# Wp-Zhang/HandyRec

Measured on NVIDIA B200. Metric: DeepFM train samples/s, higher is better.
Workload: dtype f32

## Files before the change

handyrec_b200/csrc/embedding_bwd.cu:

```cuda
#include <cub/block/block_radix_sort.cuh>
#include <cub/block/block_scan.cuh>

#include <stdlib.h>

#include <algorithm>
#include <new>
#include <vector>

#include "plan.cuh"

namespace hrb {

constexpr int UB_THREADS = 256;
constexpr int UB_IPT = 16;
constexpr int UB_CAP = UB_THREADS * UB_IPT;
constexpr int UB_EXPECT_MAX = 3686;
constexpr int UB_MAX_COLS = 256;
constexpr int UB_MAX_BINS = 256;
constexpr int UB_BINS = 64;
constexpr int UB_STACK = 256;
constexpr int UB_WARPS = UB_THREADS / 32;
constexpr int UB_HELPERS = 4;
constexpr int UB_TILE = 4096;
constexpr int SPLIT_ROUNDS = UB_TILE / UB_WARPS / 32;
constexpr uint32_t UB_INVALID = 0xFFFFFFFFu;
constexpr uint32_t UB_NONE = 0xFFFFFFFEu;
constexpr int UB_SLICE_TARGET = 4096;
constexpr int UB_PARTIAL_LD = 32 * 4 + 4;
constexpr int UB_GATHER = 8;
constexpr int UB_APPLY = 2;

static inline size_t ub_align(size_t x, size_t a = 256) { return (x + a - 1) / a * a; }

__global__ void __launch_bounds__(256) bwd_prep_kernel(const FieldDev* __restrict__ fields, const int32_t* __restrict__ pos_field,
                                                      int32_t pos_cols, const int32_t* __restrict__ ids, int64_t ids_ld, int64_t batch,
                                                      int64_t ldT, uint32_t* __restrict__ idsT) {
  __shared__ uint32_t tile[32][33];
  const int tx = threadIdx.x & 31, ty = threadIdx.x >> 5;
  const int64_t b0 = (int64_t)blockIdx.x * 32;
  const int c0 = blockIdx.y * 32;
  const int c = c0 + tx;
  int ids_col = 0, pool = 0;
  int64_t rows = 0;
  if (c < pos_cols) {
    const FieldDev& f = fields[pos_field[c]];
    ids_col = f.ids_col + (c - f.pos_col);
    pool = f.pool;
    rows = f.rows;
  }
  for (int r = ty; r < 32; r += 8) {
    const int64_t b = b0 + r;
    uint32_t v = UB_INVALID;
    if (b < batch && c < pos_cols) {
      const int32_t id = ids[b * ids_ld + ids_col];
      const bool valid = (pool == HRB_POOL_NONE || id != 0) && id >= 0 && (int64_t)id < rows;
      if (valid) v = (uint32_t)id;
    }
    tile[r][tx] = v;
  }
  __syncthreads();
  for (int r = ty; r < 32; r += 8) {
    const int cc = c0 + r;
    const int64_t b = b0 + tx;
    if (cc < pos_cols && b < ldT) idsT[(int64_t)cc * ldT + b] = tile[tx][r];
  }
}

__global__ void __launch_bounds__(256) bwd_scale_kernel(const FieldDev* __restrict__ fields, int32_t n_fields,
                                                       const int32_t* __restrict__ ids, int64_t ids_ld, int64_t batch,
                                                       float* __restrict__ scale) {
  const int64_t total = batch * n_fields;
  for (int64_t i = blockIdx.x * (int64_t)blockDim.x + threadIdx.x; i < total; i += (int64_t)gridDim.x * blockDim.x) {
    const int64_t b = i / n_fields;
    const int fi = (int)(i - b * n_fields);
    const FieldDev& f = fields[fi];
    float s = 1.0f;
    if (f.pool == HRB_POOL_MEAN) {
      const int32_t* idp = ids + b * ids_ld + f.ids_col;
      int cnt = 0;
      for (int l = 0; l < f.seq_len; ++l) {
        const int32_t id = idp[l];
        cnt += (id != 0 && id >= 0 && (int64_t)id < f.rows);
      }
      s = cnt > 0 ? __fdiv_rn(1.0f, (float)cnt) : 0.f;
    }
    scale[i] = s;
  }
}

struct SplitArgs {
  const TableSplitDev* splits;
  const TileDev* tiles;
  const uint32_t* idsT;
  int64_t ldT;
  uint32_t* tile_cnt;
  uint32_t* list_cnt;
  uint32_t* list_off;
  uint32_t* ent_row;
  uint32_t* ent_pos;
};

template <bool SCATTER>
__global__ void __launch_bounds__(UB_THREADS) split_kernel(SplitArgs a) {
  __shared__ uint32_t wcnt[UB_WARPS][UB_MAX_BINS];
  const int tid = threadIdx.x, lane = tid & 31, w = tid >> 5;
  const TileDev tile = a.tiles[blockIdx.x];
  const TableSplitDev ts = a.splits[tile.table];
  for (int i = tid; i < UB_WARPS * UB_MAX_BINS; i += UB_THREADS) (&wcnt[0][0])[i] = 0;
  __syncthreads();
  const uint32_t* colp = a.idsT + (int64_t)tile.pos_col * a.ldT;
  const int64_t b0 = (int64_t)tile.chunk * UB_TILE + w * (UB_TILE / UB_WARPS);
  uint32_t packed[SPLIT_ROUNDS];
  uint32_t idv[SPLIT_ROUNDS];
#pragma unroll
  for (int k = 0; k < SPLIT_ROUNDS; ++k) {
    const int64_t b = b0 + k * 32 + lane;
    idv[k] = b < a.ldT ? __ldg(colp + b) : UB_INVALID;
  }
#pragma unroll
  for (int k = 0; k < SPLIT_ROUNDS; ++k) {
    const uint32_t id = idv[k];
    const uint32_t bin = id == UB_INVALID ? UB_INVALID : id >> ts.shift;
    const uint32_t peers = __match_any_sync(0xffffffffu, bin);
    const int leader = __ffs(peers) - 1;
    uint32_t base = 0;
    if (bin != UB_INVALID && lane == leader) {
      base = wcnt[w][bin];
      wcnt[w][bin] = base + __popc(peers);
    }
    if (SCATTER) {
      base = __shfl_sync(0xffffffffu, base, leader);
      packed[k] = bin == UB_INVALID ? UB_INVALID : (bin << 16) | (base + __popc(peers & ((1u << lane) - 1u)));
    }
    __syncwarp();
  }
  __syncthreads();
  uint32_t* tc = a.tile_cnt + (size_t)blockIdx.x * UB_MAX_BINS;
  if (!SCATTER) {
    for (int u = tid; u < ts.n_bins; u += UB_THREADS) {
      uint32_t t = 0;
#pragma unroll
      for (int ww = 0; ww < UB_WARPS; ++ww) t += wcnt[ww][u];
      tc[u] = t;
    }
    return;
  }
  for (int u = tid; u < ts.n_bins; u += UB_THREADS) {
    uint32_t run = tc[u];
#pragma unroll
    for (int ww = 0; ww < UB_WARPS; ++ww) {
      const uint32_t t = wcnt[ww][u];
      wcnt[ww][u] = run;
      run += t;
    }
  }
  __syncthreads();
  const uint32_t mask = (1u << ts.shift) - 1u;
#pragma unroll
  for (int k = 0; k < SPLIT_ROUNDS; ++k) {
    if (packed[k] == UB_INVALID) continue;
    const int64_t b = b0 + k * 32 + lane;
    const uint32_t id = idv[k];
    const uint32_t dst = wcnt[w][packed[k] >> 16] + (packed[k] & 0xFFFFu);
    a.ent_row[dst] = id & mask;
    a.ent_pos[dst] = ((uint32_t)tile.col_local << 24) | (uint32_t)b;
  }
}

__global__ void __launch_bounds__(UB_MAX_BINS) split_scan_kernel(SplitArgs a) {
  __shared__ uint32_t tot[UB_MAX_BINS];
  const TableSplitDev ts = a.splits[blockIdx.x];
  const int u = threadIdx.x;
  uint32_t run = 0;
  if (u < ts.n_bins) {
    for (int t = 0; t < ts.n_tiles; ++t) {
      uint32_t* p = a.tile_cnt + (size_t)(ts.first_tile + t) * UB_MAX_BINS + u;
      const uint32_t c = *p;
      *p = run;
      run += c;
    }
  }
  tot[u] = u < ts.n_bins ? run : 0;
  __syncthreads();
  for (int off = 1; off < UB_MAX_BINS; off <<= 1) {
    const uint32_t v = u >= off ? tot[u - off] : 0;
    __syncthreads();
    tot[u] += v;
    __syncthreads();
  }
  if (u < ts.n_bins) {
    const uint32_t base = ts.ent_base + tot[u] - run;
    a.list_cnt[ts.first_list + u] = run;
    a.list_off[ts.first_list + u] = base;
    for (int t = 0; t < ts.n_tiles; ++t) a.tile_cnt[(size_t)(ts.first_tile + t) * UB_MAX_BINS + u] += base;
  }
}

struct UnitArgs {
  const UnitDev* units;
  const TableDev* tables;
  const ColDev* cols;
  const int32_t* col_start;
  const uint32_t* list_cnt;
  const uint32_t* list_off;
  const uint32_t* ent_row;
  const uint32_t* ent_pos;
  const float* dout;
  int64_t dout_ld;
  const float* scale;
  int32_t n_fields;
  int32_t n_units;
  hrb_opt_params opt;
  float lr_t;
  float* partials;
  int32_t debug;
};
#ifdef HRB_DEVTOOLS
#define HRB_UDBG(b) (a.debug & (b))
#else
#define HRB_UDBG(b) 0
#endif

template <int G>
struct UnitSmem {
  typedef cub::BlockRadixSort<uint32_t, UB_THREADS, UB_IPT, uint32_t> Sort;
  uint32_t row[UB_CAP];
  uint32_t pos[UB_CAP];
  union {
    typename Sort::TempStorage sort;
    float4 red[UB_THREADS];
  } u;
  ColDev cols[UB_MAX_COLS];
  int hist[UB_BINS];
  int wcnt[UB_WARPS];
  uint32_t st_lo[UB_STACK], st_hi[UB_STACK];
  int sp;
  float4 stage_acc[UB_WARPS][32 * UB_GATHER];
  uint32_t stage_row[UB_WARPS][(32 / G) * UB_GATHER];
  float4 head_acc[UB_WARPS][G], tail_acc[UB_WARPS][G];
  uint32_t head_row[UB_WARPS], tail_row[UB_WARPS];
  int head_valid[UB_WARPS], tail_valid[UB_WARPS], single[UB_WARPS];
};

template <int G>
__device__ __forceinline__ float4 unit_load_grad(const UnitArgs& a, const ColDev* cols, uint32_t packed, int q) {
  const uint32_t b = packed & 0xFFFFFFu;
  const ColDev c = cols[packed >> 24];
  float4 v = ldg_nc_na(reinterpret_cast<const float4*>(a.dout + (int64_t)b * a.dout_ld + c.out_col) + q);
  if (a.scale != nullptr) {
    const float s = __ldg(a.scale + (int64_t)b * a.n_fields + c.field);
    v.x *= s; v.y *= s; v.z *= s; v.w *= s;
  }
  return v;
}

template <int G>
__device__ int unit_compact(UnitSmem<G>& s, const uint32_t* __restrict__ lrow, const uint32_t* __restrict__ lpos, int i_lo, int i_hi,
                            uint32_t lo, uint32_t hi) {
  const int tid = threadIdx.x, lane = tid & 31, w = tid >> 5;
  const uint32_t span = hi - lo;
  const int stripe = ((i_hi - i_lo + UB_WARPS - 1) / UB_WARPS + 31) / 32 * 32;
  const int w_lo = min(i_hi, i_lo + stripe * w), w_hi = min(i_hi, w_lo + stripe);
  int cnt = 0;
  for (int i0 = w_lo; i0 < w_hi; i0 += 32 * 4) {
    uint32_t v[4];
#pragma unroll
    for (int k = 0; k < 4; ++k) {
      const int i = i0 + k * 32 + lane;
      v[k] = i < w_hi ? __ldg(lrow + i) : UB_INVALID;
    }
#pragma unroll
    for (int k = 0; k < 4; ++k) cnt += (v[k] - lo) < span;
  }
#pragma unroll
  for (int o = 16; o > 0; o >>= 1) cnt += __shfl_xor_sync(0xffffffffu, cnt, o);
  __syncthreads();
  if (lane == 0) s.wcnt[w] = cnt;
  __syncthreads();
  int base = 0, total = 0;
#pragma unroll
  for (int ww = 0; ww < UB_WARPS; ++ww) {
    const int c = s.wcnt[ww];
    if (ww < w) base += c;
    total += c;
  }
  if (total > UB_CAP || total == 0) return total;
  for (int i0 = w_lo; i0 < w_hi; i0 += 32) {
    const int i = i0 + lane;
    const uint32_t v = i < w_hi ? __ldg(lrow + i) : UB_INVALID;
    const bool hit = (v - lo) < span;
    const uint32_t bal = __ballot_sync(0xffffffffu, hit);
    if (hit) {
      const int o = base + __popc(bal & ((1u << lane) - 1u));
      s.row[o] = v - lo;
      s.pos[o] = __ldg(lpos + i);
    }
    base += __popc(bal);
  }
  return total;
}

template <int MODE, int G>
__device__ void unit_sort_reduce(UnitSmem<G>& s, const UnitArgs& a, const TableDev& T, int m, int64_t row0, uint32_t key_end) {
  constexpr int E = 32 / G;
  constexpr int U = UB_GATHER;
  const int tid = threadIdx.x;
  __syncthreads();
  if (m > 1 && !HRB_UDBG(1)) {
    uint32_t k[UB_IPT], v[UB_IPT];
#pragma unroll
    for (int j = 0; j < UB_IPT; ++j) {
      const int i = tid * UB_IPT + j;
      k[j] = i < m ? s.row[i] : key_end - 1;
      v[j] = i < m ? s.pos[i] : 0u;
    }
    int bits = 1;
    while (bits < 32 && ((key_end - 1) >> bits) != 0) ++bits;
    __syncthreads();
    typename UnitSmem<G>::Sort(s.u.sort).Sort(k, v, 0, bits);
    __syncthreads();
#pragma unroll
    for (int j = 0; j < UB_IPT; ++j) {
      const int i = tid * UB_IPT + j;
      if (i < m) {
        s.row[i] = k[j];
        s.pos[i] = v[j];
      }
    }
  }
  __syncthreads();
  const int lane = tid & 31, w = tid >> 5, e = lane / G, q = lane % G;
  const int per = ((m + UB_WARPS - 1) / UB_WARPS + E - 1) / E * E;
  const int seg_lo = w * per;
  const int seg_hi = min(m, seg_lo + per);
  if (lane == 0) {
    s.head_valid[w] = 0;
    s.tail_valid[w] = 0;
    s.single[w] = 0;
  }
  uint32_t head_row = UB_NONE;
  if (w > 0 && seg_lo < seg_hi && s.row[seg_lo - 1] == s.row[seg_lo]) head_row = s.row[seg_lo];
  uint32_t carry_row = UB_NONE;
  float4 carry = make_float4(0.f, 0.f, 0.f, 0.f);
  int stage_n = 0;
  auto close = [&](bool closing, uint32_t r, const float4& v) {
    const bool head = closing && r == head_row;
    if (head) {
      s.head_acc[w][q] = v;
// ... 193 lines not shown

template <int MODE, int G>
__global__ void __launch_bounds__(UB_THREADS, 2) bwd_unit_kernel(UnitArgs a, int unit_base) {
  extern __shared__ __align__(16) unsigned char smem_raw[];
  UnitSmem<G>& s = *reinterpret_cast<UnitSmem<G>*>(smem_raw);
  const int tid = threadIdx.x;
  const int helper = blockIdx.x / a.n_units;
  const UnitDev unit = a.units[unit_base + blockIdx.x % a.n_units];
  const int cnt = (int)a.list_cnt[unit.list];
  if (helper > 0 && (cnt <= UB_CAP || unit.n_slices > 1 || unit.row_hi - unit.row_lo == 1)) return;
  if (cnt == 0) {
    if (unit.n_slices > 1 && tid == 0) a.partials[(size_t)(unit.partial_idx + unit.slice) * UB_PARTIAL_LD + 32 * 4] = 0.f;
    return;
  }
  const uint32_t* lrow = a.ent_row + a.list_off[unit.list];
  const uint32_t* lpos = a.ent_pos + a.list_off[unit.list];
  const TableDev T = a.tables[unit.table];
  const int c0 = a.col_start[unit.table];
  const int ncol = a.col_start[unit.table + 1] - c0;
  for (int i = tid; i < ncol; i += UB_THREADS) s.cols[i] = a.cols[c0 + i];
  __syncthreads();
  const uint32_t span = unit.row_hi - unit.row_lo;
  if (unit.n_slices > 1) {
    const int i_lo = (int)((int64_t)cnt * unit.slice / unit.n_slices), i_hi = (int)((int64_t)cnt * (unit.slice + 1) / unit.n_slices);
    float4 sum;
    const int n = unit_single_row<G>(s, a, lrow, lpos, i_lo, i_hi, UB_INVALID, sum);
    float* p = a.partials + (size_t)(unit.partial_idx + unit.slice) * UB_PARTIAL_LD;
    if (tid < G) reinterpret_cast<float4*>(p)[tid] = sum;
    if (tid == 0) p[32 * 4] = (float)n;
    return;
  }
  if (span == 1) {
    float4 sum;
    unit_single_row<G>(s, a, lrow, lpos, 0, cnt, UB_INVALID, sum);
    if (tid < G) apply_table_row<MODE>(T, a.opt, a.lr_t, (int64_t)unit.row_lo, tid, sum);
    return;
  }
  if (cnt <= UB_CAP) {
    for (int i = tid; i < cnt; i += UB_THREADS) {
      s.row[i] = __ldg(lrow + i);
      s.pos[i] = __ldg(lpos + i);
    }
    if (HRB_UDBG(8)) return;
    unit_sort_reduce<MODE, G>(s, a, T, cnt, (int64_t)unit.row_lo, span);
    return;
  }
  {
    const uint32_t width = (span + UB_BINS - 1) / UB_BINS;
    unit_histogram<G>(s, lrow, cnt, 0, span, width);
    if (tid == 0) {
      int64_t before = 0;
      uint32_t my_lo = span, my_hi = 0;
      int mine = 0;
      for (int bin = 0; bin < UB_BINS; ++bin) {
        const uint32_t blo = (uint32_t)bin * width;
        if (blo >= span) break;
        const int c = s.hist[bin];
        if (c > 0 && (int)(before * UB_HELPERS / cnt) == helper) {
          my_lo = min(my_lo, blo);
          my_hi = max(my_hi, min(span, blo + width));
          mine += c;
        }
        before += c;
      }
      s.sp = 0;
      if (mine > 0) {
        s.st_lo[0] = my_lo;
        s.st_hi[0] = my_hi | (mine > UB_CAP ? 0x80000000u : 0u);
        s.sp = 1;
      }
    }
    __syncthreads();
  }
  while (true) {
    const int sp = s.sp;
    if (sp == 0) break;
    const uint32_t lo = s.st_lo[sp - 1];
    const uint32_t hi_raw = s.st_hi[sp - 1];
    const uint32_t hi = hi_raw & 0x7FFFFFFFu;
    __syncthreads();
    if (tid == 0) s.sp = sp - 1;
    if (!(hi_raw & 0x80000000u)) {
      const int m = unit_compact<G>(s, lrow, lpos, 0, cnt, lo, hi);
      if (m <= UB_CAP) {
        if (m > 0) unit_sort_reduce<MODE, G>(s, a, T, m, (int64_t)unit.row_lo + lo, hi - lo);
        __syncthreads();
        continue;
      }
    }
    if (hi - lo == 1) {
      float4 sum;
      const int n = unit_single_row<G>(s, a, lrow, lpos, 0, cnt, lo, sum);
      if (n > 0 && tid < G) apply_table_row<MODE>(T, a.opt, a.lr_t, (int64_t)unit.row_lo + lo, tid, sum);
      __syncthreads();
      continue;
    }
    const uint32_t sub = hi - lo;
    const uint32_t width = (sub + UB_BINS - 1) / UB_BINS;
    unit_histogram<G>(s, lrow, cnt, lo, hi, width);
    if (tid == 0) {
      int top = s.sp;
      int acc = 0;
      uint32_t start = lo;
      for (int bin = 0; bin < UB_BINS; ++bin) {
        const uint32_t blo = lo + (uint32_t)bin * width;
        if (blo >= hi) break;
        const uint32_t bhi = min(hi, blo + width);
        const int c = s.hist[bin];
        if (c > UB_CAP) {
          if (acc > 0 && top < UB_STACK) { s.st_lo[top] = start; s.st_hi[top] = blo; ++top; }
          if (top < UB_STACK) { s.st_lo[top] = blo; s.st_hi[top] = bhi | 0x80000000u; ++top; }
          start = bhi;
          acc = 0;
        } else if (acc + c > UB_CAP) {
          if (top < UB_STACK) { s.st_lo[top] = start; s.st_hi[top] = blo; ++top; }
          start = blo;
          acc = c;
        } else {
          acc += c;
        }
      }
      if (acc > 0 && top < UB_STACK) { s.st_lo[top] = start; s.st_hi[top] = hi; ++top; }
      s.sp = top;
    }
    __syncthreads();
  }
}

template <int MODE, int G>
__global__ void __launch_bounds__(256) bwd_unit_combine_kernel(UnitArgs a, const SliceGroupDev* __restrict__ groups, int group_base, int n_groups) {
  const int gi = blockIdx.x * (blockDim.x / G) + threadIdx.x / G, q = threadIdx.x % G;
  if (gi >= n_groups) return;
  const SliceGroupDev sg = groups[group_base + gi];
  float4 acc = make_float4(0.f, 0.f, 0.f, 0.f);
  float n = 0.f;
  for (int sl = 0; sl < sg.n_slices; ++sl) {
    const float* p = a.partials + (size_t)(sg.partial_idx + sl) * UB_PARTIAL_LD;
    const float cnt = p[32 * 4];
    if (cnt > 0.f) {
      const float4 v = reinterpret_cast<const float4*>(p)[q];
      acc.x += v.x; acc.y += v.y; acc.z += v.z; acc.w += v.w;
    }
    n += cnt;
  }
  if (n > 0.f) apply_table_row<MODE>(a.tables[sg.table], a.opt, a.lr_t, (int64_t)sg.row, q, acc);
}

struct UnitHost {
  UnitDev d;
  int32_t g;
  int64_t expect;
};

static inline int64_t unit_ldT(int64_t batch) { return (batch + 15) / 16 * 16; }

static int build_units(const hrb_plan* plan, int64_t batch) {
  UnitSet& us = plan->units;
  if (us.batch == batch) return HRB_OK;
  us.ok = false;
  us.batch = batch;
  std::vector<UnitHost> units;
  std::vector<SliceGroupDev> groups;
  std::vector<int32_t> group_g;
  std::vector<TableSplitDev> splits(plan->n_tables);
  std::vector<TileDev> tiles;
  int32_t n_partials = 0, n_lists = 0;
  const int64_t n_chunks = (unit_ldT(batch) + UB_TILE - 1) / UB_TILE;
  std::vector<int32_t> col_pos;
  for (int t = 0; t < plan->n_tables; ++t)
    for (int f = 0; f < plan->n_fields; ++f) {
      if (plan->fields[f].table != t) continue;
      for (int l = 0; l < plan->fields[f].seq_len; ++l) col_pos.push_back(plan->fdev_host[f].pos_col + l);
    }
  for (int t = 0; t < plan->n_tables; ++t) {
    const TableDev& td = plan->tdev_host[t];
    const int64_t ncol = plan->col_start_host[t + 1] - plan->col_start_host[t];
    TableSplitDev& sp = splits[t];
    sp = TableSplitDev{n_lists, 0, 0, (int32_t)tiles.size(), 0, (uint32_t)(batch * plan->col_start_host[t])};
    if (ncol == 0) continue;
    const int64_t n_t = batch * ncol;
    int shift = 0;
    while (shift < 31 && (int64_t)(2ll << shift) * n_t <= (int64_t)UB_EXPECT_MAX * td.rows) ++shift;
    const int64_t range = 1ll << shift;
    const int64_t n_bins = (td.rows + range - 1) / range;
    if (n_bins > UB_MAX_BINS) return HRB_OK;
    sp.n_bins = (int32_t)n_bins;
    sp.shift = shift;
    sp.n_tiles = (int32_t)(ncol * n_chunks);
    for (int64_t cl = 0; cl < ncol; ++cl)
      for (int64_t ch = 0; ch < n_chunks; ++ch)
        tiles.push_back(TileDev{t, (int32_t)cl, col_pos[plan->col_start_host[t] + cl], (int32_t)ch});
    const int32_t g = td.dim / 4;
    for (int64_t bin = 0; bin < n_bins; ++bin) {
      const int64_t lo = bin * range, hi = std::min<int64_t>(td.rows, lo + range);
      const int64_t expect = n_t * (hi - lo) / td.rows;
      UnitHost u{};
      u.d.table = t;
      u.d.row_lo = (uint32_t)lo;
      u.d.row_hi = (uint32_t)hi;
      u.d.n_slices = 1;
      u.d.list = n_lists + (int32_t)bin;
      u.g = g;
      u.expect = expect;
      if (hi - lo == 1 && expect > 2 * UB_SLICE_TARGET) {
        int64_t ns = (expect + UB_SLICE_TARGET - 1) / UB_SLICE_TARGET;
        if (ns > 64) ns = 64;
        groups.push_back(SliceGroupDev{t, (uint32_t)lo, n_partials, (int32_t)ns});
        group_g.push_back(g);
        for (int64_t sl = 0; sl < ns; ++sl) {
          UnitHost v = u;
          v.d.slice = (int32_t)sl;
          v.d.n_slices = (int32_t)ns;
          v.d.partial_idx = n_partials;
          v.expect = expect / ns;
          units.push_back(v);
        }
        n_partials += (int32_t)ns;
      } else {
        units.push_back(u);
      }
    }
    n_lists += (int32_t)n_bins;
  }
  std::stable_sort(units.begin(), units.end(), [](const UnitHost& x, const UnitHost& y) {
    if (x.g != y.g) return x.g < y.g;
    return x.expect > y.expect;
  });
  std::vector<size_t> gorder(groups.size());
  for (size_t i = 0; i < gorder.size(); ++i) gorder[i] = i;
  std::stable_sort(gorder.begin(), gorder.end(), [&](size_t x, size_t y) { return group_g[x] < group_g[y]; });
  std::vector<UnitDev> ud(units.size());
  std::vector<SliceGroupDev> gd(groups.size());
  us.n_g = 0;
  for (size_t i = 0; i < units.size(); ++i) {
    ud[i] = units[i].d;
    if (us.n_g == 0 || us.g_values[us.n_g - 1] != units[i].g) {
      if (us.n_g >= 8) return fail(HRB_UNSUPPORTED, "embedding backward: more than 8 distinct embedding dims in one plan");
      us.g_values[us.n_g] = units[i].g;
      us.g_unit_off[us.n_g] = (int32_t)i;
      ++us.n_g;
    }
  }
  us.g_unit_off[us.n_g] = (int32_t)units.size();
  for (size_t i = 0; i < gorder.size(); ++i) gd[i] = groups[gorder[i]];
  us.g_group_off[0] = 0;
  for (int gi = 0; gi < us.n_g; ++gi) {
    int32_t cnt = 0;
    for (size_t i = 0; i < group_g.size(); ++i) cnt += group_g[i] == us.g_values[gi];
    us.g_group_off[gi + 1] = us.g_group_off[gi] + cnt;
  }
  if (us.d_blob) cudaFree(us.d_blob);
  us.d_blob = nullptr;
  const size_t sz_u = ub_align(sizeof(UnitDev) * (ud.size() + 1)), sz_g = ub_align(sizeof(SliceGroupDev) * (gd.size() + 1));
  const size_t sz_s = ub_align(sizeof(TableSplitDev) * (splits.size() + 1)), sz_t = ub_align(sizeof(TileDev) * (tiles.size() + 1));
  HRB_CUDA(cudaMalloc(&us.d_blob, sz_u + sz_g + sz_s + sz_t));
  char* d = (char*)us.d_blob;
  if (!ud.empty()) HRB_CUDA(cudaMemcpy(d, ud.data(), sizeof(UnitDev) * ud.size(), cudaMemcpyHostToDevice));
  if (!gd.empty()) HRB_CUDA(cudaMemcpy(d + sz_u, gd.data(), sizeof(SliceGroupDev) * gd.size(), cudaMemcpyHostToDevice));
  HRB_CUDA(cudaMemcpy(d + sz_u + sz_g, splits.data(), sizeof(TableSplitDev) * splits.size(), cudaMemcpyHostToDevice));
  if (!tiles.empty()) HRB_CUDA(cudaMemcpy(d + sz_u + sz_g + sz_s, tiles.data(), sizeof(TileDev) * tiles.size(), cudaMemcpyHostToDevice));
  us.d_units = (UnitDev*)d;
  us.d_groups = (SliceGroupDev*)(d + sz_u);
  us.d_splits = (TableSplitDev*)(d + sz_u + sz_g);
  us.d_tiles = (TileDev*)(d + sz_u + sz_g + sz_s);
  us.n_units = (int32_t)ud.size();
  us.n_groups = (int32_t)gd.size();
  us.n_partials = n_partials;
  us.n_lists = n_lists;
  us.n_tiles = (int32_t)tiles.size();
  us.ok = true;
  return HRB_OK;
}

bool unit_path_supported(const hrb_plan* plan, int64_t batch) {
  if (!(plan->unit_path_ok && !plan->has_max && batch < (1ll << 24) && batch > 0)) return false;
  std::lock_guard<std::mutex> lock(plan->unit_mu);
  return build_units(plan, batch) == HRB_OK && plan->units.ok;
}

struct UnitWs {
  size_t idsT, scale, partials, ent_row, ent_pos, tile_cnt, list_cnt, list_off, total;
};
static UnitWs carve_unit_ws(const hrb_plan* plan, int64_t batch) {
  const UnitSet& us = plan->units;
  UnitWs w{};
  size_t off = 0;
  auto take = [&](size_t bytes) {
    const size_t o = off;
    off += ub_align(bytes);
    return o;
  };
  const size_t n = (size_t)batch * plan->pos_cols;
  w.idsT = take((size_t)plan->pos_cols * unit_ldT(batch) * 4);
  w.scale = take((size_t)batch * plan->n_fields * 4 + 4);
  w.partials = take((size_t)(us.n_partials + 1) * UB_PARTIAL_LD * 4);
  w.ent_row = take(n * 4 + 4);
  w.ent_pos = take(n * 4 + 4);
  w.tile_cnt = take((size_t)(us.n_tiles + 1) * UB_MAX_BINS * 4);
  w.list_cnt = take((size_t)(us.n_lists + 1) * 4);
  w.list_off = take((size_t)(us.n_lists + 1) * 4);
  w.total = off;
  return w;
}

size_t unit_workspace_bytes(const hrb_plan* plan, int64_t batch) {
  std::lock_guard<std::mutex> lock(plan->unit_mu);
  return carve_unit_ws(plan, batch).total;
}

template <int MODE, int G>
static int launch_units(UnitArgs a, const UnitSet& us, int gi, cudaStream_t st) {
  static bool attr = false;
  const size_t smem = sizeof(UnitSmem<G>);
  if (!attr) {
    HRB_CUDA(cudaFuncSetAttribute(bwd_unit_kernel<MODE, G>, cudaFuncAttributeMaxDynamicSharedMemorySize, (int)smem));
    attr = true;
  }
  const int n = us.g_unit_off[gi + 1] - us.g_unit_off[gi];
  if (n > 0) {
    a.n_units = n;
    bwd_unit_kernel<MODE, G><<<n * (HRB_UDBG(32) ? 1 : UB_HELPERS), UB_THREADS, smem, st>>>(a, us.g_unit_off[gi]);
    HRB_LAUNCH_CHECK();
  }
  const int ng = us.g_group_off[gi + 1] - us.g_group_off[gi];
  if (ng > 0) {
    const int gpb = 256 / G;
    bwd_unit_combine_kernel<MODE, G><<<(ng + gpb - 1) / gpb, 256, 0, st>>>(a, us.d_groups, us.g_group_off[gi], ng);
    HRB_LAUNCH_CHECK();
  }
  return HRB_OK;
}

int run_unit_update(const hrb_plan* plan, const int32_t* ids, int64_t ids_ld, int64_t batch, const float* dout, int64_t dout_ld,
                    const hrb_opt_params& opt, void* workspace, size_t workspace_bytes, cudaStream_t st) {
  std::lock_guard<std::mutex> lock(plan->unit_mu);
  int rc = build_units(plan, batch);
  if (rc != HRB_OK) return rc;
  const UnitSet& us = plan->units;
  if (!us.ok) return fail(HRB_UNSUPPORTED, "embedding backward: unit path not available for this plan / batch");
  const UnitWs ws = carve_unit_ws(plan, batch);
  if (ws.total > workspace_bytes) return fail(HRB_WORKSPACE, "hrb_lookup_bwd_update: workspace %zu < required %zu bytes", workspace_bytes, ws.total);
  char* base = (char*)workspace;
  const int64_t ldT = unit_ldT(batch);
  uint32_t* idsT = (uint32_t*)(base + ws.idsT);
  float* scale = (float*)(base + ws.scale);
  dim3 pg((unsigned)((ldT + 31) / 32), (unsigned)((plan->pos_cols + 31) / 32));
  bwd_prep_kernel<<<pg, 256, 0, st>>>(plan->d_fields, plan->d_pos_field, plan->pos_cols, ids, ids_ld, batch, ldT, idsT);
  HRB_LAUNCH_CHECK();
  if (plan->has_mean) {
    int64_t blocks = (batch * plan->n_fields + 255) / 256;
    const int64_t cap = (int64_t)sm_count() * 8;
    if (blocks > cap) blocks = cap;
    bwd_scale_kernel<<<(unsigned)blocks, 256, 0, st>>>(plan->d_fields, plan->n_fields, ids, ids_ld, batch, scale);
    HRB_LAUNCH_CHECK();
  }
  SplitArgs sa{us.d_splits, us.d_tiles, idsT, ldT, (uint32_t*)(base + ws.tile_cnt), (uint32_t*)(base + ws.list_cnt),
               (uint32_t*)(base + ws.list_off), (uint32_t*)(base + ws.ent_row), (uint32_t*)(base + ws.ent_pos)};
  if (us.n_tiles > 0) {
    split_kernel<false><<<us.n_tiles, UB_THREADS, 0, st>>>(sa);
    HRB_LAUNCH_CHECK();
    split_scan_kernel<<<plan->n_tables, UB_MAX_BINS, 0, st>>>(sa);
    HRB_LAUNCH_CHECK();
    split_kernel<true><<<us.n_tiles, UB_THREADS, 0, st>>>(sa);
    HRB_LAUNCH_CHECK();
  }
  UnitArgs a{};
  a.units = us.d_units;
  a.tables = plan->d_tables;
  a.cols = plan->d_cols;
  a.col_start = plan->d_col_start;
  a.list_cnt = sa.list_cnt;
  a.list_off = sa.list_off;
  a.ent_row = sa.ent_row;
  a.ent_pos = sa.ent_pos;
  a.dout = dout;
  a.dout_ld = dout_ld;
  a.scale = plan->has_mean ? scale : nullptr;
  a.n_fields = plan->n_fields;
  a.opt = opt;
  a.lr_t = opt.opt == HRB_OPT_ADAM_LAZY ? opt.lr * sqrtf(opt.bias_corr2) / opt.bias_corr1 : 0.f;
  a.partials = (float*)(base + ws.partials);
#ifdef HRB_DEVTOOLS
  {
    static int dbg = -1;
    if (dbg < 0) {
      const char* e = getenv("HRB_BWD_DEBUG");
      dbg = e ? atoi(e) : 0;
    }
    a.debug = dbg;
  }
#endif
  const int mode = upd_mode(opt.opt);
  for (int gi = 0; gi < us.n_g; ++gi) {
#define HRB_UNITS(GG)                                                                      \
  rc = mode == UPD_ADAM      ? launch_units<UPD_ADAM, GG>(a, us, gi, st)                   \
       : mode == UPD_ADAGRAD ? launch_units<UPD_ADAGRAD, GG>(a, us, gi, st)                \
       : mode == UPD_FTRL    ? launch_units<UPD_FTRL, GG>(a, us, gi, st)                   \
                             : launch_units<UPD_SGD, GG>(a, us, gi, st);                   \
  break;
    switch (us.g_values[gi]) {
      case 1: HRB_UNITS(1)
      case 2: HRB_UNITS(2)
      case 4: HRB_UNITS(4)
      case 8: HRB_UNITS(8)
      case 16: HRB_UNITS(16)
      case 32: HRB_UNITS(32)
      default: rc = fail(HRB_UNSUPPORTED, "embedding backward: dim %d", us.g_values[gi] * 4);
    }
#undef HRB_UNITS
    if (rc != HRB_OK) return rc;
  }
  return HRB_OK;
}

}
```

handyrec_b200/csrc/lookup.cu:

```cuda
#include <cub/device/device_radix_sort.cuh>
#include <algorithm>
#include <new>
#include <stdlib.h>
#include <string.h>
#include <vector>

#include "common.cuh"

#include "plan.cuh"

namespace hrb {

constexpr uint32_t kNotMine = 0xFFFFFFFFu;

__global__ void __launch_bounds__(256) embedding_fwd_kernel(const float* __restrict__ table, int64_t vocab,
                                                            int32_t chunks ,
                                                            const int32_t* __restrict__ ids, int64_t n_ids,
                                                            float* __restrict__ out, uint8_t* __restrict__ mask,
                                                            int32_t* __restrict__ oob) {
  const int64_t total = n_ids * chunks;
  const int64_t stride = (int64_t)gridDim.x * blockDim.x;
  constexpr int U = 4;
  for (int64_t base = blockIdx.x * (int64_t)blockDim.x + threadIdx.x; base < total; base += stride * U) {
    int32_t id[U];
// ... 1141 lines not shown
  if (rc != HRB_OK) return rc;
  if (batch == 0) return HRB_OK;
  if (inv_count == nullptr && plan->all_len1 && plan->uniform_dim && plan->contiguous_out) {
    const int G = plan->max_dim / 4;
    if (G == 2 || G == 4 || G == 8 || G == 16)
      return launch_rows<false>(plan, ids, ids_ld, batch, out, out_ld, nullptr, nullptr, nullptr, nullptr, nullptr, oob, (cudaStream_t)stream);
  }
  const unsigned grid = grid_for(batch * plan->out_chunks, 256, 8);
  lookup_items_kernel<false><<<grid, 256, 0, (cudaStream_t)stream>>>(plan->d_fields, plan->d_chunk_field,
                                                                    plan->d_chunk_q, plan->out_chunks, plan->n_fields,
                                                                    ids, ids_ld, batch, out, out_ld, inv_count, oob);
  HRB_LAUNCH_CHECK();
  return HRB_OK;
}

HRB_API int hrb_lookup_fm_fwd(const hrb_plan* plan, const int32_t* ids, int64_t ids_ld, int64_t batch, float* out,
                              int64_t out_ld, float* inv_count, const float* fm_w, const float* fm_w0, float* fm_out,
                              float* fm_sum, int32_t* oob, void* stream) {
  int rc = check_lookup_args("hrb_lookup_fm_fwd", plan, ids, ids_ld, batch, out, out_ld);
  if (rc != HRB_OK) return rc;
  HRB_REQUIRE(fm_w && fm_w0 && fm_out, "hrb_lookup_fm_fwd: fm_w / fm_w0 / fm_out is NULL");
  HRB_REQUIRE(aligned16(fm_w) && (fm_sum == nullptr || aligned16(fm_sum)), "hrb_lookup_fm_fwd: fm_w/fm_sum must be 16-byte aligned");
  if (!plan->uniform_dim)
    return fail(HRB_UNSUPPORTED, "hrb_lookup_fm_fwd: FM needs every field to have the same embedding dim");
  if (batch == 0) return HRB_OK;
  return launch_rows<true>(plan, ids, ids_ld, batch, out, out_ld, inv_count, fm_w, fm_w0, fm_out, fm_sum, oob,
                           (cudaStream_t)stream);
}

constexpr int MARK_MAX_TABLES = 512;
struct TouchedPtrs {
  float* p[MARK_MAX_TABLES];
};

__global__ void __launch_bounds__(256) mark_rows_kernel(const FieldDev* __restrict__ fields, int32_t n_fields, const int32_t* __restrict__ ids,
                                                       int64_t ids_ld, int64_t batch, const TouchedPtrs tp) {
  const int64_t total = batch * n_fields;
  for (int64_t i = blockIdx.x * (int64_t)blockDim.x + threadIdx.x; i < total; i += (int64_t)gridDim.x * blockDim.x) {
    const int64_t b = i / n_fields;
    const FieldDev& f = fields[i - b * n_fields];
    float* touched = tp.p[f.table_idx];
    if (touched == nullptr) continue;
    const int32_t* idp = ids + b * ids_ld + f.ids_col;
    for (int l = 0; l < f.seq_len; ++l) {
      const int32_t id = idp[l];
      if (id >= 0 && (int64_t)id < f.rows) touched[id] = 1.0f;
    }
  }
}

__global__ void __launch_bounds__(256) pad_flags_kernel(const FieldDev* __restrict__ fields, int32_t n_fields, const int32_t* __restrict__ ids,
                                                       int64_t ids_ld, int64_t batch, float* __restrict__ flags) {
  const int64_t total = batch * n_fields;
  for (int64_t i = blockIdx.x * (int64_t)blockDim.x + threadIdx.x; i < total; i += (int64_t)gridDim.x * blockDim.x) {
    const int64_t b = i / n_fields;
    const FieldDev& f = fields[i - b * n_fields];
    const int32_t* idp = ids + b * ids_ld + f.ids_col;
    bool zero = false;
    for (int l = 0; l < f.seq_len; ++l) zero |= idp[l] == 0;
    float* fl = flags + 2 * f.table_idx + (f.pool == HRB_POOL_NONE ? 1 : 0);
    if (zero && *fl == 0.f) *fl = 1.0f;
  }
}

__global__ void __launch_bounds__(256) ftrl_pad_kernel(const TableDev* __restrict__ tables, int32_t n_tables, const float* __restrict__ flags,
                                                      const hrb_opt_params opt) {
  for (int32_t ti = 0; ti < n_tables; ++ti) {
    const TableDev& t = tables[ti];
    if (t.grad != nullptr || flags[2 * ti] == 0.f || flags[2 * ti + 1] != 0.f) continue;
    for (int e = threadIdx.x; e < t.dim; e += blockDim.x) {
      const float w = t.w[e];
      float a = t.m[e], l = t.v[e];
      t.w[e] = ftrl_elem(w, a, l, fmaf(opt.l2_scale, w, 0.f), opt.lr, opt.l1, opt.l2, opt.lr_power, opt.l2_shrinkage);
      t.m[e] = a;
      t.v[e] = l;
    }
  }
}

static bool has_pooled(const hrb_plan* plan) {
  for (const auto& f : plan->fdev_host)
    if (f.pool != HRB_POOL_NONE) return true;
  return false;
}
static size_t pad_flag_bytes(const hrb_plan* plan) { return has_pooled(plan) ? align_up((size_t)plan->n_tables * 8) : 0; }

static int ftrl_tables_ok(const hrb_plan* plan, const char* who) {
  for (const auto& t : plan->tdev_host)
    HRB_REQUIRE(t.grad || (t.m && t.v), "%s: Ftrl needs an accumulator (adam_m) and a linear slot (adam_v) for every row-updated table", who);
  return HRB_OK;
}

static int launch_pad_flags(const hrb_plan* plan, const int32_t* ids, int64_t ids_ld, int64_t batch, float* flags, cudaStream_t st) {
  HRB_CUDA(cudaMemsetAsync(flags, 0, (size_t)plan->n_tables * 8, st));
  pad_flags_kernel<<<grid_for(batch * plan->n_fields, 256), 256, 0, st>>>(plan->d_fields, plan->n_fields, ids, ids_ld, batch, flags);
  HRB_LAUNCH_CHECK();
  return HRB_OK;
}

static int launch_ftrl_pad(const hrb_plan* plan, const float* flags, const hrb_opt_params& opt, cudaStream_t st) {
  ftrl_pad_kernel<<<1, 256, 0, st>>>(plan->d_tables, plan->n_tables, flags, opt);
  HRB_LAUNCH_CHECK();
  return HRB_OK;
}

HRB_API int hrb_plan_mark_rows(const hrb_plan* plan, const int32_t* ids, int64_t ids_ld, int64_t batch, float* const* touched_host,
                               void* stream) {
  HRB_REQUIRE(plan && ids && touched_host && batch >= 0, "hrb_plan_mark_rows: null/negative argument");
  if (plan->n_tables > MARK_MAX_TABLES) return fail(HRB_UNSUPPORTED, "hrb_plan_mark_rows: more than %d tables", MARK_MAX_TABLES);
  TouchedPtrs tp{};
  bool any = false;
  for (int32_t t = 0; t < plan->n_tables; ++t) {
    tp.p[t] = touched_host[t];
    any |= touched_host[t] != nullptr;
  }
  if (batch == 0 || !any) return HRB_OK;
  mark_rows_kernel<<<grid_for(batch * plan->n_fields, 256), 256, 0, (cudaStream_t)stream>>>(plan->d_fields, plan->n_fields, ids, ids_ld,
                                                                                           batch, tp);
  HRB_LAUNCH_CHECK();
  return HRB_OK;
}

HRB_API int hrb_plan_pad_flags(const hrb_plan* plan, const int32_t* ids, int64_t ids_ld, int64_t batch, float* flags, void* stream) {
  HRB_REQUIRE(plan && ids && flags && batch >= 0, "hrb_plan_pad_flags: null/negative argument");
  if (batch == 0) return HRB_OK;
  pad_flags_kernel<<<grid_for(batch * plan->n_fields, 256), 256, 0, (cudaStream_t)stream>>>(plan->d_fields, plan->n_fields, ids, ids_ld,
                                                                                           batch, flags);
  HRB_LAUNCH_CHECK();
  return HRB_OK;
}

HRB_API int hrb_plan_ftrl_pad_step(const hrb_plan* plan, const float* flags, const hrb_opt_params* opt_host, void* stream) {
  HRB_REQUIRE(plan && flags && opt_host, "hrb_plan_ftrl_pad_step: null argument");
  HRB_REQUIRE(opt_host->opt == HRB_OPT_FTRL, "hrb_plan_ftrl_pad_step: needs HRB_OPT_FTRL, got %d", opt_host->opt);
  int rc = ftrl_tables_ok(plan, "hrb_plan_ftrl_pad_step");
  if (rc != HRB_OK) return rc;
  return launch_ftrl_pad(plan, flags, load_opt(opt_host), (cudaStream_t)stream);
}

HRB_API int hrb_lookup_bwd_workspace(const hrb_plan* plan, int64_t ids_ld, int64_t batch, size_t* bytes) {
  HRB_REQUIRE(plan && bytes && batch >= 0, "hrb_lookup_bwd_workspace: null/negative argument");
  (void)ids_ld;
  const int64_t n = batch * plan->pos_cols;
  HRB_REQUIRE(n < 0x7FFFFFFFll, "hrb_lookup_bwd_workspace: batch*sum(seq_len) = %lld exceeds 2^31-1", (long long)n);
  BwdWorkspace w;
  int rc = carve_bwd_ws(n > 0 ? n : 1, batch * plan->n_fields + 1, plan->max_dim, plan->key_bits, nullptr, w);
  if (rc != HRB_OK) return rc;
  *bytes = w.total;
  if (unit_path_supported(plan, batch)) *bytes = std::max(w.total, unit_workspace_bytes(plan, batch));
  if (const size_t fb = pad_flag_bytes(plan)) *bytes = align_up(*bytes) + fb;
  return HRB_OK;
}

static int run_plan_sorted_update(const hrb_plan* plan, const int32_t* ids, int64_t ids_ld, int64_t batch, const float* dout,
                                  int64_t dout_ld, const hrb_opt_params& opt, void* workspace, size_t workspace_bytes, cudaStream_t st);

HRB_API int hrb_lookup_bwd_update(const hrb_plan* plan, const int32_t* ids, int64_t ids_ld, int64_t batch,
                                  const float* dout, int64_t dout_ld, const float* inv_count,
                                  const hrb_opt_params* opt_host, void* workspace, size_t workspace_bytes,
                                  void* stream) {
  (void)inv_count;
  HRB_REQUIRE(plan && ids && dout && opt_host && workspace && batch >= 0, "hrb_lookup_bwd_update: null/negative argument");
  HRB_REQUIRE(aligned16(dout) && dout_ld % 4 == 0, "hrb_lookup_bwd_update: dout must be 16-byte aligned, dout_ld %% 4 == 0");
  if (plan->has_max)
    return fail(HRB_UNSUPPORTED, "hrb_lookup_bwd_update: max-pooled fields go through hrb_seq_pool_bwd + hrb_embedding_bwd_dense");
  const hrb_opt_params opt = load_opt(opt_host);
  HRB_REQUIRE(opt.opt == HRB_OPT_SGD || opt.opt == HRB_OPT_ADAM_LAZY || opt.opt == HRB_OPT_ADAGRAD || opt.opt == HRB_OPT_FTRL,
              "hrb_lookup_bwd_update: unknown optimiser %d", opt.opt);
  if (opt.opt == HRB_OPT_ADAM_LAZY)
    for (const auto& t : plan->tdev_host)
      HRB_REQUIRE(t.grad || (t.m && t.v), "hrb_lookup_bwd_update: lazy Adam needs adam_m/adam_v for every table");
  if (opt.opt == HRB_OPT_ADAGRAD)
    for (const auto& t : plan->tdev_host)
      HRB_REQUIRE(t.grad || t.m, "hrb_lookup_bwd_update: Adagrad needs an accumulator (adam_m) for every row-updated table");
  if (opt.opt == HRB_OPT_FTRL) {
    int rc = ftrl_tables_ok(plan, "hrb_lookup_bwd_update");
    if (rc != HRB_OK) return rc;
  }
  const int G = plan->max_dim / 4;
  if (G > 256) return fail(HRB_UNSUPPORTED, "hrb_lookup_bwd_update: dim %d too large", plan->max_dim);
  if (batch == 0) return HRB_OK;
  const int64_t n = batch * plan->pos_cols;
  HRB_REQUIRE(n < 0x7FFFFFFFll, "hrb_lookup_bwd_update: batch*sum(seq_len) exceeds 2^31-1");
  cudaStream_t st = (cudaStream_t)stream;
  float* pad_flags = nullptr;
  if (opt.opt == HRB_OPT_FTRL && has_pooled(plan)) {
    const size_t fb = pad_flag_bytes(plan);
    if (workspace_bytes < fb) return fail(HRB_WORKSPACE, "hrb_lookup_bwd_update: workspace %zu < %zu bytes of padding flags", workspace_bytes, fb);
    workspace_bytes = (workspace_bytes - fb) / 256 * 256;
    pad_flags = (float*)((char*)workspace + workspace_bytes);
    int rc = launch_pad_flags(plan, ids, ids_ld, batch, pad_flags, st);
    if (rc != HRB_OK) return rc;
  }
  int rc = HRB_OK;
  if (plan->bwd_algo != HRB_BWD_SORT && unit_path_supported(plan, batch))
    rc = run_unit_update(plan, ids, ids_ld, batch, dout, dout_ld, opt, workspace, workspace_bytes, st);
  else
    rc = run_plan_sorted_update(plan, ids, ids_ld, batch, dout, dout_ld, opt, workspace, workspace_bytes, st);
  if (rc != HRB_OK || pad_flags == nullptr) return rc;
  return launch_ftrl_pad(plan, pad_flags, opt, st);
}

static int run_plan_sorted_update(const hrb_plan* plan, const int32_t* ids, int64_t ids_ld, int64_t batch, const float* dout,
                                  int64_t dout_ld, const hrb_opt_params& opt, void* workspace, size_t workspace_bytes, cudaStream_t st) {
  const int G = plan->max_dim / 4;
  const int64_t n = batch * plan->pos_cols;
  BwdWorkspace w;
  int rc = carve_bwd_ws(n, batch * plan->n_fields + 1, plan->max_dim, plan->key_bits, workspace, w);
  if (rc != HRB_OK) return rc;
  if (w.total > workspace_bytes)
    return fail(HRB_WORKSPACE, "hrb_lookup_bwd_update: workspace %zu < required %zu bytes", workspace_bytes, w.total);
  const uint32_t sentinel = (uint32_t)plan->total_rows;
  bwd_keys_kernel<<<grid_for(batch * plan->n_fields, 256), 256, 0, st>>>(plan->d_fields, plan->n_fields, plan->pos_cols,
                                                                        ids, ids_ld, batch, sentinel, w.keys_in,
                                                                        w.vals_in, w.scale);
  HRB_LAUNCH_CHECK();
  PlanGrad src{plan->d_fields, plan->d_pos_field, dout, w.scale, dout_ld, plan->pos_cols, plan->n_fields};
  ApplyCtx ctx{plan->d_tables, plan->n_tables, opt, nullptr, 0.f};
  if (opt.opt == HRB_OPT_ADAM_LAZY)
    ctx.lr_t = opt.lr * sqrtf(opt.bias_corr2) / opt.bias_corr1;
  return run_sorted_update(upd_mode(opt.opt), w, n, sentinel, plan->key_bits, G, src, ctx, hot_from_plan(plan), st);
}

HRB_API int hrb_embedding_bwd_dense_workspace(int64_t n_ids, int32_t dim, size_t* bytes) {
  HRB_REQUIRE(bytes && n_ids >= 0 && dim > 0, "hrb_embedding_bwd_dense_workspace: bad argument");
  HRB_REQUIRE(n_ids < 0x7FFFFFFFll, "hrb_embedding_bwd_dense_workspace: n_ids exceeds 2^31-1");
  BwdWorkspace w;
  int rc = carve_bwd_ws(n_ids > 0 ? n_ids : 1, 1, dim, 32, nullptr, w);
  if (rc != HRB_OK) return rc;
  *bytes = w.total + align_up(sizeof(TableDev));
  return HRB_OK;
}

HRB_API int hrb_embedding_bwd_dense(const int32_t* ids, int64_t n_ids, const float* dout, int64_t vocab, int32_t dim,
                                    const float* table, float l2_scale, float* dtable, void* workspace,
                                    size_t workspace_bytes, void* stream) {
  HRB_REQUIRE(ids && dout && dtable && workspace && n_ids >= 0 && vocab > 0 && dim > 0, "hrb_embedding_bwd_dense: null/negative argument");
  if (dim % 4 != 0) return fail(HRB_UNSUPPORTED, "hrb_embedding_bwd_dense: dim %d is not a multiple of 4", dim);
  HRB_REQUIRE(aligned16(dout) && aligned16(dtable), "hrb_embedding_bwd_dense: dout/dtable must be 16-byte aligned");
  HRB_REQUIRE(vocab < 0xFFFFFFFFll && n_ids < 0x7FFFFFFFll, "hrb_embedding_bwd_dense: sizes exceed 32-bit keys");
  cudaStream_t st = (cudaStream_t)stream;
  dense_grad_init_kernel<<<grid_for(vocab * dim, 256), 256, 0, st>>>(l2_scale != 0.f ? table : nullptr, l2_scale,
                                                                    vocab * (int64_t)dim, dtable);
  HRB_LAUNCH_CHECK();
  if (n_ids == 0) return HRB_OK;
  const int key_bits = bits_for((uint64_t)vocab);
  BwdWorkspace w;
  int rc = carve_bwd_ws(n_ids, 1, dim, key_bits, workspace, w);
  if (rc != HRB_OK) return rc;
  const size_t need = w.total + align_up(sizeof(TableDev));
  if (need > workspace_bytes)
    return fail(HRB_WORKSPACE, "hrb_embedding_bwd_dense: workspace %zu < required %zu bytes", workspace_bytes, need);
  TableDev* d_t = (TableDev*)((char*)workspace + w.total);
  TableDev t{dtable, nullptr, nullptr, vocab, 0u, dim};
  HRB_CUDA(cudaMemcpyAsync(d_t, &t, sizeof(t), cudaMemcpyHostToDevice, st));
  const uint32_t sentinel = (uint32_t)vocab;
  flat_keys_kernel<<<grid_for(n_ids, 256), 256, 0, st>>>(ids, n_ids, vocab, sentinel, w.keys_in, w.vals_in);
  HRB_LAUNCH_CHECK();
  FlatGrad src{dout, dim};
  ApplyCtx ctx{d_t, 1, hrb_opt_params{}, dtable, 0.f};
  HotInfo hot{};
  if (vocab <= HOT_MAX_ROWS) {
    hot.n_ranges = 1;
    hot.lo[0] = 0;
    hot.len[0] = (uint32_t)vocab;
    hot.keys = nullptr;
    hot.n_keys = (int32_t)vocab;
  }
  return run_sorted_update(UPD_DENSE_ADD, w, n_ids, sentinel, key_bits, dim / 4, src, ctx, hot, st);
}

namespace hrb {

__device__ __forceinline__ bool routed_id_valid(const FieldDev& f, int32_t id, const int64_t* __restrict__ full_rows) {
  return (f.pool == HRB_POOL_NONE || id != 0) && id >= 0 && (full_rows == nullptr || (int64_t)id < full_rows[f.table_idx]);
}

__global__ void __launch_bounds__(256) route_kernel(const FieldDev* __restrict__ fields, const int32_t* __restrict__ pos_field,
                                                   int32_t pos_cols, const int32_t* __restrict__ ids, int64_t ids_ld, int64_t batch,
                                                   int32_t n_ranks, const uint32_t* __restrict__ key_base ,
                                                   int32_t n_tables, const int64_t* __restrict__ full_rows, uint32_t* __restrict__ owner,
                                                   uint32_t* __restrict__ key, uint32_t* __restrict__ pos) {
  const int64_t total = batch * pos_cols;
  for (int64_t i = blockIdx.x * (int64_t)blockDim.x + threadIdx.x; i < total; i += (int64_t)gridDim.x * blockDim.x) {
    const int64_t b = i / pos_cols;
    const int c = (int)(i - b * pos_cols);
    const FieldDev& f = fields[pos_field[c]];
    const int32_t id = ids[b * ids_ld + f.ids_col + (c - f.pos_col)];
    const bool valid = routed_id_valid(f, id, full_rows);
    const uint32_t o = valid ? (uint32_t)(id % n_ranks) : (uint32_t)n_ranks;
    owner[i] = o;
    key[i] = valid ? key_base[o * n_tables + f.table_idx] + (uint32_t)(id / n_ranks) : 0xFFFFFFFFu;
    pos[i] = (uint32_t)i;
  }
}

__global__ void owner_counts_kernel(const uint32_t* __restrict__ sorted_owner, int64_t n, int32_t n_ranks,
                                    int64_t* __restrict__ counts) {
  const int r = blockIdx.x * blockDim.x + threadIdx.x;
  if (r > n_ranks) return;
  auto lower = [&](uint32_t v) {
    int64_t lo = 0, hi = n;
    while (lo < hi) {
      const int64_t mid = (lo + hi) >> 1;
      if (sorted_owner[mid] < v) lo = mid + 1; else hi = mid;
    }
    return lo;
  };
  counts[r] = lower((uint32_t)r + 1) - lower((uint32_t)r);
}

__global__ void __launch_bounds__(256) gather_u32_kernel(const uint32_t* __restrict__ src, const uint32_t* __restrict__ perm,
                                                        int64_t n, uint32_t* __restrict__ dst) {
  for (int64_t i = blockIdx.x * (int64_t)blockDim.x + threadIdx.x; i < n; i += (int64_t)gridDim.x * blockDim.x)
    dst[i] = src[perm[i]];
}

__global__ void __launch_bounds__(256) rows_by_key_kernel(const TableDev* __restrict__ tables, int32_t n_tables, int32_t chunks,
                                                         const uint32_t* __restrict__ keys, int64_t n, float* __restrict__ out) {
  const int64_t total = n * chunks;
  for (int64_t i = blockIdx.x * (int64_t)blockDim.x + threadIdx.x; i < total; i += (int64_t)gridDim.x * blockDim.x) {
    const int64_t j = i / chunks;
    const int q = (int)(i - j * chunks);
    const uint32_t k = __ldg(keys + j);
    const int ti = find_table(tables, n_tables, k);
    const TableDev& t = tables[ti];
    const int64_t row = (int64_t)(k - t.key_base);
    float4 v = make_float4(0.f, 0.f, 0.f, 0.f);
    if (row < t.rows && q * 4 < t.dim) v = ldg_nc_na(reinterpret_cast<const float4*>(t.w) + row * (t.dim >> 2) + q);
    stg_na(reinterpret_cast<float4*>(out) + i, v);
  }
}

__global__ void __launch_bounds__(256) scatter_rows_kernel(const FieldDev* __restrict__ fields, const int32_t* __restrict__ pos_field,
                                                          int32_t pos_cols, int32_t chunks, const uint32_t* __restrict__ perm,
                                                          int64_t n, const float* __restrict__ rows, float* __restrict__ out,
                                                          int64_t out_ld, float* __restrict__ pos_rows) {
  const int64_t total = n * chunks;
  for (int64_t i = blockIdx.x * (int64_t)blockDim.x + threadIdx.x; i < total; i += (int64_t)gridDim.x * blockDim.x) {
    const int64_t j = i / chunks;
    const int q = (int)(i - j * chunks);
    const uint32_t p = __ldg(perm + j);
    const int64_t b = p / (uint32_t)pos_cols;
    const int c = (int)(p - (uint32_t)b * (uint32_t)pos_cols);
    const FieldDev& f = fields[__ldg(pos_field + c)];
    const float4 v = __ldg(reinterpret_cast<const float4*>(rows) + i);
    if (f.pool == HRB_POOL_NONE)
      *(reinterpret_cast<float4*>(out + b * out_ld + f.out_col) + q) = v;
    else
      *(reinterpret_cast<float4*>(pos_rows) + (int64_t)p * chunks + q) = v;
  }
}

__global__ void __launch_bounds__(256) pool_positions_kernel(const FieldDev* __restrict__ fields, int32_t n_fields, int32_t pos_cols,
                                                            int32_t chunks, const int32_t* __restrict__ ids, int64_t ids_ld,
                                                            int64_t batch, const float* __restrict__ pos_rows,
                                                            float* __restrict__ out, int64_t out_ld, const int64_t* __restrict__ full_rows) {
  const int64_t total = batch * n_fields * chunks;
  for (int64_t i = blockIdx.x * (int64_t)blockDim.x + threadIdx.x; i < total; i += (int64_t)gridDim.x * blockDim.x) {
    const int q = (int)(i % chunks);
    const int64_t bf = i / chunks;
    const int fi = (int)(bf % n_fields);
    const int64_t b = bf / n_fields;
    const FieldDev& f = fields[fi];
// ... 309 lines not shown
```

handyrec_b200/csrc/plan.cuh:

```cuda
#pragma once
#include <cstddef>
#include <mutex>
#include <vector>

#include "common.cuh"

namespace hrb {

struct FieldDev {
  const float* table;
  int64_t rows;
  uint32_t key_base;
  int32_t dim;
  int32_t seq_len;
  int32_t pool;
  int32_t ids_col;
  int32_t out_col;
  int32_t pos_col;
  int32_t table_idx;
};

struct TableDev {
  float* w;
  float* m;
// ... 41 lines not shown
  if (t.grad != nullptr) {
    float4* gp = reinterpret_cast<float4*>(t.grad) + off;
    float4 o = *gp;
    o.x += g.x; o.y += g.y; o.z += g.z; o.w += g.w;
    *gp = o;
    return;
  }
  float4* wp = reinterpret_cast<float4*>(t.w) + off;
  float4 w = *wp;
  if (MODE == UPD_FTRL) {
    float4* ap = reinterpret_cast<float4*>(t.m) + off;
    float4* lp = reinterpret_cast<float4*>(t.v) + off;
    float4 a = *ap, l = *lp;
    const float l2 = opt.l2_scale;
    g.x = fmaf(l2, w.x, g.x); g.y = fmaf(l2, w.y, g.y); g.z = fmaf(l2, w.z, g.z); g.w = fmaf(l2, w.w, g.w);
    ftrl_row4(w, a, l, g, opt);
    *ap = a;
    *lp = l;
    *wp = w;
    return;
  }
  const float l2 = opt.l2_scale;
  g.x = fmaf(l2, w.x, g.x); g.y = fmaf(l2, w.y, g.y); g.z = fmaf(l2, w.z, g.z); g.w = fmaf(l2, w.w, g.w);
  if (MODE == UPD_SGD) {
    const float lr = opt.lr;
    w.x -= lr * g.x; w.y -= lr * g.y; w.z -= lr * g.z; w.w -= lr * g.w;
  } else if (MODE == UPD_ADAGRAD) {
    float4* ap = reinterpret_cast<float4*>(t.m) + off;
    float4 a = *ap;
    const float lr = opt.lr, e = opt.eps;
    adagrad_elem(w.x, a.x, g.x, lr, e); adagrad_elem(w.y, a.y, g.y, lr, e);
    adagrad_elem(w.z, a.z, g.z, lr, e); adagrad_elem(w.w, a.w, g.w, lr, e);
    *ap = a;
  } else {
    float4* mp = reinterpret_cast<float4*>(t.m) + off;
    float4* vp = reinterpret_cast<float4*>(t.v) + off;
    float4 m = *mp, v = *vp;
    const float b1 = opt.beta1, b2 = opt.beta2, e = opt.eps, lr = lr_t;
    m.x = b1 * m.x + (1.f - b1) * g.x; m.y = b1 * m.y + (1.f - b1) * g.y;
    m.z = b1 * m.z + (1.f - b1) * g.z; m.w = b1 * m.w + (1.f - b1) * g.w;
    v.x = b2 * v.x + (1.f - b2) * g.x * g.x; v.y = b2 * v.y + (1.f - b2) * g.y * g.y;
    v.z = b2 * v.z + (1.f - b2) * g.z * g.z; v.w = b2 * v.w + (1.f - b2) * g.w * g.w;
    w.x -= lr * m.x / (sqrtf(v.x) + e); w.y -= lr * m.y / (sqrtf(v.y) + e);
    w.z -= lr * m.z / (sqrtf(v.z) + e); w.w -= lr * m.w / (sqrtf(v.w) + e);
    *mp = m;
    *vp = v;
  }
  *wp = w;
}

template <int MODE, int N>
__device__ __forceinline__ void apply_table_rows(const TableDev& t, const hrb_opt_params& opt, float lr_t, const int64_t (&row)[N],
                                                 const bool (&ok_in)[N], int q, float4 (&g)[N]) {
  const bool in_dim = q * 4 < t.dim;
  bool ok[N];
  int64_t off[N];
#pragma unroll
  for (int i = 0; i < N; ++i) {
    ok[i] = ok_in[i] && in_dim;
    off[i] = row[i] * (t.dim >> 2) + q;
  }
  if (t.grad != nullptr) {
    float4 o[N];
#pragma unroll
    for (int i = 0; i < N; ++i)
      if (ok[i]) o[i] = reinterpret_cast<float4*>(t.grad)[off[i]];
#pragma unroll
    for (int i = 0; i < N; ++i)
      if (ok[i]) {
        o[i].x += g[i].x; o[i].y += g[i].y; o[i].z += g[i].z; o[i].w += g[i].w;
        reinterpret_cast<float4*>(t.grad)[off[i]] = o[i];
      }
    return;
  }
  float4 w[N], m[N], v[N];
#pragma unroll
  for (int i = 0; i < N; ++i) {
    if (ok[i]) {
      w[i] = reinterpret_cast<float4*>(t.w)[off[i]];
      if (MODE != UPD_SGD) m[i] = reinterpret_cast<float4*>(t.m)[off[i]];
      if (MODE == UPD_ADAM || MODE == UPD_FTRL) v[i] = reinterpret_cast<float4*>(t.v)[off[i]];
    }
  }
  const float l2 = opt.l2_scale;
#pragma unroll
  for (int i = 0; i < N; ++i) {
    if (!ok[i]) continue;
    float4 gi = g[i], wi = w[i];
    gi.x = fmaf(l2, wi.x, gi.x); gi.y = fmaf(l2, wi.y, gi.y); gi.z = fmaf(l2, wi.z, gi.z); gi.w = fmaf(l2, wi.w, gi.w);
    if (MODE == UPD_SGD) {
      const float lr = opt.lr;
      wi.x -= lr * gi.x; wi.y -= lr * gi.y; wi.z -= lr * gi.z; wi.w -= lr * gi.w;
    } else if (MODE == UPD_ADAGRAD) {
      float4 ai = m[i];
      const float lr = opt.lr, e = opt.eps;
      adagrad_elem(wi.x, ai.x, gi.x, lr, e); adagrad_elem(wi.y, ai.y, gi.y, lr, e);
      adagrad_elem(wi.z, ai.z, gi.z, lr, e); adagrad_elem(wi.w, ai.w, gi.w, lr, e);
      reinterpret_cast<float4*>(t.m)[off[i]] = ai;
    } else if (MODE == UPD_FTRL) {
      float4 ai = m[i], li = v[i];
      ftrl_row4(wi, ai, li, gi, opt);
      reinterpret_cast<float4*>(t.m)[off[i]] = ai;
      reinterpret_cast<float4*>(t.v)[off[i]] = li;
    } else {
      float4 mi = m[i], vi = v[i];
      const float b1 = opt.beta1, b2 = opt.beta2, e = opt.eps, lr = lr_t;
      mi.x = b1 * mi.x + (1.f - b1) * gi.x; mi.y = b1 * mi.y + (1.f - b1) * gi.y;
      mi.z = b1 * mi.z + (1.f - b1) * gi.z; mi.w = b1 * mi.w + (1.f - b1) * gi.w;
      vi.x = b2 * vi.x + (1.f - b2) * gi.x * gi.x; vi.y = b2 * vi.y + (1.f - b2) * gi.y * gi.y;
      vi.z = b2 * vi.z + (1.f - b2) * gi.z * gi.z; vi.w = b2 * vi.w + (1.f - b2) * gi.w * gi.w;
      wi.x -= lr * mi.x / (sqrtf(vi.x) + e); wi.y -= lr * mi.y / (sqrtf(vi.y) + e);
      wi.z -= lr * mi.z / (sqrtf(vi.z) + e); wi.w -= lr * mi.w / (sqrtf(vi.w) + e);
      reinterpret_cast<float4*>(t.m)[off[i]] = mi;
      reinterpret_cast<float4*>(t.v)[off[i]] = vi;
    }
    reinterpret_cast<float4*>(t.w)[off[i]] = wi;
  }
}

struct UnitDev {
  int32_t table;
  uint32_t row_lo, row_hi;
  int32_t slice, n_slices;
  int32_t partial_idx;
  int32_t list;
  int32_t pad_;
};
struct ColDev {
  int32_t pos_col;
  int32_t out_col;
  int32_t field;
  int32_t pad_;
};
struct SliceGroupDev {
  int32_t table;
  uint32_t row;
  int32_t partial_idx, n_slices;
};
struct TableSplitDev {
  int32_t first_list, n_bins, shift;
  int32_t first_tile, n_tiles;
  uint32_t ent_base;
};
struct TileDev {
  int32_t table, col_local, pos_col, chunk;
};
struct UnitSet {
  int64_t batch = -1;
  void* d_blob = nullptr;
  UnitDev* d_units = nullptr;
  SliceGroupDev* d_groups = nullptr;
  TableSplitDev* d_splits = nullptr;
  TileDev* d_tiles = nullptr;
  int32_t n_units = 0, n_groups = 0, n_partials = 0, n_lists = 0, n_tiles = 0;
  int32_t g_values[8] = {0};
  int32_t g_unit_off[9] = {0};
  int32_t g_group_off[9] = {0};
  int32_t n_g = 0;
  bool ok = false;
};

}

struct hrb_plan {
  int32_t n_tables = 0, n_fields = 0;
  std::vector<hrb_table_desc> tables;
  std::vector<hrb_field_desc> fields;
  std::vector<hrb::FieldDev> fdev_host;
  std::vector<hrb::TableDev> tdev_host;
  uint64_t total_rows = 0;
  int key_bits = 1;
  int32_t pos_cols = 0;
  int32_t out_chunks = 0;
  int32_t max_dim = 0;
  bool uniform_dim = true;
  bool contiguous_out = true;
  bool all_len1 = true;
  bool has_max = false;
  void* dev_blob = nullptr;
  hrb::FieldDev* d_fields = nullptr;
  hrb::TableDev* d_tables = nullptr;
  int32_t* d_chunk_field = nullptr;
  int32_t* d_chunk_q = nullptr;
  int32_t* d_pos_field = nullptr;
  uint32_t* d_hot_keys = nullptr;
  int32_t n_hot_keys = 0;
  std::vector<uint32_t> hot_lo, hot_len;
  int32_t n_ranks = 1;
  const float** d_peer_tab = nullptr;
  int64_t* d_full_rows = nullptr;
  hrb::ColDev* d_cols = nullptr;
  int32_t* d_col_start = nullptr;
  std::vector<int32_t> col_start_host;
  bool unit_path_ok = false;
  bool has_mean = false;
  int32_t bwd_algo = 0;
  mutable std::mutex unit_mu;
  mutable hrb::UnitSet units;
};


namespace hrb {
bool unit_path_supported(const hrb_plan* plan, int64_t batch);
size_t unit_workspace_bytes(const hrb_plan* plan, int64_t batch);
int run_unit_update(const hrb_plan* plan, const int32_t* ids, int64_t ids_ld, int64_t batch, const float* dout, int64_t dout_ld,
                    const hrb_opt_params& opt, void* workspace, size_t workspace_bytes, cudaStream_t st);
}
```

handyrec_b200/engine.py:

```python
from __future__ import annotations

import ctypes
import math
from typing import Dict, List, Optional, Sequence, Tuple

import numpy as np
import torch

from . import _lib
from . import kernels as K
from ._lib import call


def _r4(n: int) -> int:
    return (n + 3) // 4 * 4


def launch_count() -> int:
    c = ctypes.c_int64(0)
    call("hrb_launch_count", ctypes.byref(c))
    return c.value


class DeepFMEngine:
# ... 144 lines not shown
        self.dZ = [torch.zeros(B, ld, **f32) for ld in self.layer_ld]
        self.dX0 = torch.zeros(B, self.K0p, **f32)
        self.fm_out = torch.empty(B, **f32)
        self.fm_sum = torch.empty(B, self.D, **f32)
        self.prob = torch.empty(B, **f32)
        self.loss_sum = torch.zeros(1, **f32)
        self.use_tc = gemm_mode != _lib.GEMM_FP32 and B >= 512 and B % 4 == 0
        self.tc_layer = [self.use_tc and u >= 16 for u in self.units]
        if self.use_tc:
            self.Wt = [torch.zeros(ld, Kp, **f32) if tc else None for ld, Kp, tc in zip(self.layer_ld, self.layer_K, self.tc_layer)]
            self.dZt = [torch.zeros(ld, B, **f32) for ld in self.layer_ld]
            self.relu_mask = [torch.zeros(B, (u + 31) // 32, device=self.dev, dtype=torch.int32) if self.act == "relu" else None for u in self.units]
            self._refresh_wt()
        self.ids_dev = torch.zeros(B, self.ids_cols, device=self.dev, dtype=torch.int32)
        self.dense_dev = torch.zeros(B, max(self.n_dense, 1), **f32)
        self.label_dev = torch.zeros(B, **f32)
        self.loss_host = torch.zeros(1, dtype=torch.float32).pin_memory()
        self._ws_emb = torch.empty(self.plan.workspace_bytes(B), device=self.dev, dtype=torch.uint8)

    _n_pad_flags = 0
    metrics = None

    _marks = None

    _timeline = None

    def _mark(self, name: str) -> None:
        if self._timeline is not None:
            e = torch.cuda.Event(enable_timing=True)
            e.record()
            self._timeline.append((name, e))
        if self._marks is not None:
            e = torch.cuda.Event(enable_timing=True)
            e.record()
            self._marks.append((name, e))

    def profile_step(self, ids, dense, label) -> "OrderedDict[str, float]":
        from collections import OrderedDict

        self._marks = []
        self._mark("start")
        self.train_step_on_device(ids, dense, label)
        torch.cuda.current_stream().synchronize()
        marks, self._marks = self._marks, None
        out = OrderedDict()
        for (n0, e0), (n1, e1) in zip(marks[:-1], marks[1:]):
            out[n1] = out.get(n1, 0.0) + e0.elapsed_time(e1)
        return out

    def timeline_step(self, ids, dense, label) -> "OrderedDict[str, float]":
        from collections import OrderedDict

        torch.cuda.synchronize()
        self._timeline = []
        self._mark("start")
        self.train_step_on_device(ids, dense, label)
        self._mark("end")
        torch.cuda.synchronize()
        tl, self._timeline = self._timeline, None
        e0 = tl[0][1]
        return OrderedDict((n, round(e0.elapsed_time(e), 4)) for n, e in tl[1:])

    def _refresh_wt(self) -> None:
        if not getattr(self, "use_tc", False):
            return
        st = K._stream()
        for i, tc in enumerate(self.tc_layer):
            if tc:
                call("hrb_transpose", K._p(self.W[i]), self.layer_K[i], self.layer_ld[i], self.layer_ld[i], K._p(self.Wt[i]), self.layer_K[i], st)

    def _init_dense(self, seed: int) -> None:
        g = torch.Generator().manual_seed(seed)
        for i, (Kl, u) in enumerate(zip(self.layer_Kl, self.units)):
            lim = math.sqrt(6.0 / (Kl + u))
            w = (torch.rand(Kl, u, generator=g) * 2 - 1) * lim
            self.set_dense_weights(i, w, torch.zeros(u))
        lim = math.sqrt(6.0 / (self.D + 1))
        self.fm_w.copy_(((torch.rand(self.D, generator=g) * 2 - 1) * lim).to(self.dev))
        self.fm_w0.zero_()

    def set_dense_weights(self, i: int, w: torch.Tensor, b: torch.Tensor) -> None:
        Kl, u = self.layer_Kl[i], self.units[i]
        assert tuple(w.shape) == (Kl, u) and tuple(b.shape) == (u,)
        W = torch.zeros(self.layer_K[i], self.layer_ld[i])
        if i == 0:
            W[: self.n_dense, :u] = w[: self.n_dense]
            W[self.nd_pad :, :u] = w[self.n_dense :]
        else:
            W[:Kl, :u] = w
        self.W[i].copy_(W.to(self.dev))
        bb = torch.zeros(self.layer_ld[i])
        bb[:u] = b
        self.b[i].copy_(bb.to(self.dev))
        self._refresh_wt()

    def get_dense_weights(self, i: int) -> Tuple[torch.Tensor, torch.Tensor]:
        Kl, u = self.layer_Kl[i], self.units[i]
        W = self.W[i].cpu()
        if i == 0:
            w = torch.cat([W[: self.n_dense, :u], W[self.nd_pad :, :u]], 0)
        else:
            w = W[:Kl, :u]
        return w.clone(), self.b[i][:u].cpu().clone()

    def get_dense_grads(self, i: int) -> Tuple[torch.Tensor, torch.Tensor]:
        Kl, u = self.layer_Kl[i], self.units[i]
        W = self.dW[i].cpu()
        w = torch.cat([W[: self.n_dense, :u], W[self.nd_pad :, :u]], 0) if i == 0 else W[:Kl, :u]
        return w.clone(), self.db[i][:u].cpu().clone()

    def forward(self, ids: torch.Tensor, dense: Optional[torch.Tensor], training: bool = False) -> torch.Tensor:
        B = ids.shape[0]
        assert B <= self.B
        st = K._stream()
        if self.n_dense:
            call("hrb_pack_dense", K._p(dense), int(dense.dtype == torch.int32), dense.stride(0), B, self.n_dense, self.nd_pad,
                 K._p(self.X0), self.K0p, st)
            self._mark("pack_dense")
        self._lookup_fm_forward(ids, B, st)
        x, ldx = self.X0, self.K0p
        n = len(self.units)
        for i in range(n):
            act = self.act if i + 1 != n else "linear"
            if self.units[i] == 1 and self.layer_K[i] % 4 == 0:
                call("hrb_dense1_fwd", K._p(x), ldx, K._p(self.W[i]), K._p(self.b[i]), B, self.layer_K[i], K._p(self.A[i]), st)
            elif self.use_tc and self.tc_layer[i] and B == self.B:
                call("hrb_dense_fwd_t", K._p(x), ldx, K._p(self.Wt[i]), self.layer_K[i], K._p(self.b[i]), B, self.layer_K[i], self.units[i],
                     _lib.ACT[act], K._p(self.A[i]), self.layer_ld[i], None, B,
                     K._p(self.relu_mask[i]) if (training and act == "relu") else None, st)
            else:
                call("hrb_dense_fwd", K._p(x), ldx, K._p(self.W[i]), self.layer_ld[i], K._p(self.b[i]), B, self.layer_K[i], self.units[i],
                     _lib.ACT[act], K._p(self.A[i]), self.layer_ld[i], _lib.GEMM_FP32, st)
            self._mark(f"dense_fwd_{i}")
            x, ldx = self.A[i], self.layer_ld[i]
        return self.A[-1]

    def _lookup_fm_forward(self, ids, B, st) -> None:
        call("hrb_lookup_fm_fwd", self.plan._h, K._p(ids), ids.stride(0), B, K._p(self.X0), self.K0p, None, K._p(self.fm_w),
             K._p(self.fm_w0), K._p(self.fm_out), K._p(self.fm_sum), None, st)
        self._mark("lookup_fm_fwd")

    def _zero_table_grads(self) -> None:
        if self.grads.numel() > self.n_dense_params:
            self.grads[self.n_dense_params :].zero_()

    def _mark_touched(self, plan, ids, tables) -> None:
        if self.touched is not None and self.l2_embd == 0.0:
            plan.mark_rows(ids, [self.table_touched[t] for t in tables])

    autotune_embedding_bwd = True
    _bwd_trials: Optional[list] = None
    bwd_algo = "auto"

    def _embedding_backward(self, ids, B, st, op) -> None:
        self._zero_table_grads()
        self._mark_touched(self.plan, ids, range(len(self.tables)))
        trial = None
        n_trials = len(self._bwd_trials or [])
        if self.autotune_embedding_bwd and self._marks is None and B == self.B and self.step_count >= 3 and n_trials < 4 and self.bwd_algo == "auto":
            trial = _lib.BWD_UNITS if n_trials % 2 == 0 else _lib.BWD_SORT
            call("hrb_plan_set_bwd_algo", self.plan._h, trial)
            e0, e1 = torch.cuda.Event(enable_timing=True), torch.cuda.Event(enable_timing=True)
            e0.record()
        call("hrb_lookup_bwd_update", self.plan._h, K._p(ids), ids.stride(0), B, K._p(self.dX0), self.K0p, None, ctypes.byref(op),
             K._p(self._ws_emb), self._ws_emb.numel(), st)
        if trial is not None:
            e1.record()
            e1.synchronize()
            self._bwd_trials = (self._bwd_trials or []) + [(trial, e0.elapsed_time(e1))]
            if len(self._bwd_trials) == 4:
                best = {}
                for algo, ms in self._bwd_trials:
                    best[algo] = min(best.get(algo, 1e30), ms)
                pick = min(best, key=best.get)
                call("hrb_plan_set_bwd_algo", self.plan._h, pick)
                self.bwd_algo = "units" if pick == _lib.BWD_UNITS else "sort"
                self.bwd_algo_ms = {("units" if a == _lib.BWD_UNITS else "sort"): round(m, 4) for a, m in best.items()}
        self._mark("embedding_bwd_update")

    def _pre_embedding_backward(self) -> None:
        """Sharded engine: finish the routing exchange (host sync on data that is ready since the forward)."""

    def _sync_dense_grads(self) -> None:
        """Replicated dense parameters: the sharded engine all-reduces the flat gradient buffer here."""

    grad_scale_div = 1
    overlap_embedding_bwd = False
    _side = None
    _side_pending = False

    def predict_on_device(self, ids: torch.Tensor, dense: Optional[torch.Tensor]) -> torch.Tensor:
        B = ids.shape[0]
        self.forward(ids, dense)
        call("hrb_sigmoid_bce", K._p(self.A[-1]), K._p(self.fm_out), K._p(self.label_dev), B, 0.0, K._p(self.prob), None, None, K._stream())
        return self.prob[:B]

    def train_step_on_device(self, ids: torch.Tensor, dense: Optional[torch.Tensor], label: torch.Tensor) -> None:
        B = ids.shape[0]
        st = K._stream()
        self.step_count += 1
        self.forward(ids, dense, training=True)
        self.loss_sum.zero_()
        dlogit = self.dZ[-1]
        call("hrb_sigmoid_bce", K._p(self.A[-1]), K._p(self.fm_out), K._p(label), B, 1.0 / (B * self.grad_scale_div), K._p(self.prob), K._p(dlogit), K._p(self.loss_sum), st)
        self._mark("sigmoid_bce")
        if self.metrics is not None:
            self.metrics.update(self.prob[:B], label)
            self._mark("metric_update")
        self._backward(ids, B, st)

    def _backward(self, ids: torch.Tensor, B: int, st) -> None:
        n = len(self.units)
        need = ctypes.c_size_t(0)
        dz, lddz = self.dZ[-1], self.layer_ld[-1]
        tc_step = self.use_tc and B == self.B
        op = _lib.OptParams()
        op.opt = {"sgd": _lib.OPT_SGD, "adagrad": _lib.OPT_ADAGRAD, "ftrl": _lib.OPT_FTRL}.get(self.emb_opt, _lib.OPT_ADAM_LAZY)
        op.lr, op.beta1, op.beta2, op.eps, op.l2_scale = self.lr, self.beta1, self.beta2, self.eps, 2.0 * self.l2_embd
        op.bias_corr1, op.bias_corr2 = 1.0 - self.beta1 ** self.step_count, 1.0 - self.beta2 ** self.step_count
        op.l1, op.l2, op.lr_power, op.l2_shrinkage = self.l1, self.ftrl_l2, self.lr_power, self.l2_shrinkage
        self._op = op
        emb_done = [False]

        def bwd_x_0(dz0, lddz0) -> None:
            Kp0, N0 = self.layer_K[0], self.units[0]
            call("hrb_dense_bwd_x_t", K._p(dz0), lddz0, K._p(self.W[0]), self.layer_ld[0], B, Kp0, N0, None, 0, 0, None, K._p(self.dX0), self.K0p,
                 None, 0, st)

        def emb_part(side: bool) -> None:
            emb_done[0] = True
            emb_x = self.X0[:, self.nd_pad :]
            emb_dx = self.dX0[:, self.nd_pad :]
            call("hrb_fm_bwd", K._p(emb_x), self.K0p, B, self.F, self.D, K._p(self.fm_w), K._p(self.dZ[-1]), K._p(emb_dx), self.K0p, 1,
                 K._p(self.d_fm), K._stream())
            self._mark("fm_bwd")
            if side and self._marks is None:
                main = torch.cuda.current_stream()
                if self._side is None:
                    self._side = torch.cuda.Stream()
                with torch.cuda.stream(self._side):
                    self._pre_embedding_backward()
                self._side.wait_stream(main)
                with torch.cuda.stream(self._side):
                    self._embedding_backward(ids, B, K._stream(), op)
                self._side_pending = True
            else:
                self._embedding_backward(ids, B, K._stream(), op)

        for i in range(n - 1, -1, -1):
            x, ldx = (self.A[i - 1], self.layer_ld[i - 1]) if i > 0 else (self.X0, self.K0p)
            Kp, N = self.layer_K[i], self.units[i]
            if N == 1 and i > 0 and Kp % 4 == 0 and Kp <= 1024:
                call("hrb_dense1_bwd_workspace", B, Kp, ctypes.byref(need))
                ws = self._dense_ws(need.value)
                call("hrb_dense1_bwd", K._p(x), ldx, K._p(self.W[i]), K._p(dz), B, Kp, _lib.ACT[self.act], K._p(self.dZ[i - 1]), self.layer_ld[i - 1],
                     K._p(self.dZt[i - 1]) if tc_step else None, B, K._p(self.dW[i]), K._p(self.db[i]), K._p(ws), ws.numel(), st)
                dz, lddz = self.dZ[i - 1], self.layer_ld[i - 1]
                self._mark(f"dense_bwd_{i}_logit")
                continue
            if tc_step and self.tc_layer[i] and i == 0 and self.overlap_embedding_bwd:
                bwd_x_0(dz, lddz)
                self._mark("dense_bwd_x_0")
                emb_part(side=True)
                call("hrb_dense_bwd_w_t_workspace", B, Kp, N, ctypes.byref(need))
                ws = self._dense_ws(need.value)
                call("hrb_dense_bwd_w_xn", K._p(self.X0), self.K0p, K._p(self.dZt[0]), B, B, Kp, N, K._p(self.dW[0]), self.layer_ld[0],
                     K._p(self.db[0]), K._p(ws), ws.numel(), st)
                self._mark("dense_bwd_w_0")
                continue
            if tc_step and self.tc_layer[i]:
                call("hrb_dense_bwd_w_t_workspace", B, Kp, N, ctypes.byref(need))
                ws = self._dense_ws(need.value)
                call("hrb_dense_bwd_w_xn", K._p(x), ldx, K._p(self.dZt[i]), B, B, Kp, N, K._p(self.dW[i]), self.layer_ld[i],
                     K._p(self.db[i]), K._p(ws), ws.numel(), st)
                self._mark(f"dense_bwd_w_{i}")
                if i > 0:
                    use_mask = self.act == "relu" and self.tc_layer[i - 1]
                    call("hrb_dense_bwd_x_t", K._p(dz), lddz, K._p(self.W[i]), self.layer_ld[i], B, Kp, N, K._p(self.A[i - 1]), self.layer_ld[i - 1],
                         _lib.ACT[self.act], K._p(self.relu_mask[i - 1]) if use_mask else None, K._p(self.dZ[i - 1]), self.layer_ld[i - 1],
                         K._p(self.dZt[i - 1]), B, st)
                    dz, lddz = self.dZ[i - 1], self.layer_ld[i - 1]
                else:
                    bwd_x_0(dz, lddz)
                self._mark(f"dense_bwd_x_{i}")
                continue
            call("hrb_dense_bwd_w_workspace", B, Kp, N, ctypes.byref(need))
            ws = self._dense_ws(need.value)
            call("hrb_dense_bwd_w", K._p(x), ldx, K._p(dz), lddz, B, Kp, N, K._p(self.dW[i]), self.layer_ld[i], K._p(self.db[i]),
                 K._p(ws), ws.numel(), _lib.GEMM_FP32, st)
            self._mark(f"dense_bwd_w_{i}")
            if i > 0:
                call("hrb_dense_bwd_x", K._p(dz), lddz, K._p(self.W[i]), self.layer_ld[i], B, Kp, N, K._p(self.A[i - 1]), self.layer_ld[i - 1],
                     _lib.ACT[self.act], K._p(self.dZ[i - 1]), self.layer_ld[i - 1], _lib.GEMM_FP32, st)
                dz, lddz = self.dZ[i - 1], self.layer_ld[i - 1]
                if tc_step:
                    call("hrb_transpose", K._p(dz), B, self.units[i - 1], lddz, K._p(self.dZt[i - 1]), B, st)
            else:
                call("hrb_dense_bwd_x", K._p(dz), lddz, K._p(self.W[0]), self.layer_ld[0], B, Kp, N, None, 0, 0, K._p(self.dX0), self.K0p,
                     _lib.GEMM_FP32, st)
            self._mark(f"dense_bwd_x_{i}")
        if not emb_done[0]:
            emb_part(side=False)
        self._sync_dense_grads()
        segs = [(o_, n_, 2.0 * self.l2_dnn if reg else 0.0) for o_, n_, reg in self._segments]
        ftrl_rows = self.optimizer == "ftrl" and self.touched is not None and self.l2_embd == 0.0
        if self.n_params > self.n_dense_params and not ftrl_rows:
            segs.append((self.n_dense_params, self.n_params - self.n_dense_params, 2.0 * self.l2_embd))
        merged = [segs[0]]
        for o_, n_, l2_ in segs[1:]:
            po, pn, pl = merged[-1]
            if pl == l2_ and po + pn == o_:
                merged[-1] = (po, pn + n_, pl)
            else:
                merged.append((o_, n_, l2_))
        for off, length, l2s in merged:
            o = off * 4
            pp = lambda t: ctypes.c_void_p(t.data_ptr() + o)
            if self.optimizer == "adam":
                call("hrb_adam_step", pp(self.params), pp(self.grads), pp(self.opt_m), pp(self.opt_v), length, self.lr, self.beta1,
                     self.beta2, self.eps, op.bias_corr1, op.bias_corr2, l2s, st)
            elif self.optimizer == "adagrad":
                call("hrb_adagrad_step", pp(self.params), pp(self.grads), pp(self.opt_m), length, self.lr, self.eps, l2s, st)
            elif self.optimizer == "ftrl":
                call("hrb_ftrl_step", pp(self.params), pp(self.grads), pp(self.opt_m), pp(self.opt_v), length, self.lr, self.l1, self.ftrl_l2,
                     self.lr_power, self.l2_shrinkage, l2s, None, 0, st)
            else:
                call("hrb_sgd_step", pp(self.params), pp(self.grads), length, self.lr, l2s, st)
        if ftrl_rows:
            o = self.tab0 * 4
            pp = lambda t: ctypes.c_void_p(t.data_ptr() + o)
            call("hrb_ftrl_step", pp(self.params), pp(self.grads), pp(self.opt_m), pp(self.opt_v), self.n_params - self.tab0, self.lr, self.l1,
                 self.ftrl_l2, self.lr_power, self.l2_shrinkage, 0.0, K._p(self.touched), self.D, st)
        self._refresh_wt()
        if self._side_pending:
            torch.cuda.current_stream().wait_stream(self._side)
            self._side_pending = False
        self._mark("dense_optimizer")

    _dws: Optional[torch.Tensor] = None

    def _dense_ws(self, nbytes: int) -> torch.Tensor:
        if self._dws is None or self._dws.numel() < nbytes:
            self._dws = torch.empty(max(nbytes, 1 << 20), device=self.dev, dtype=torch.uint8)
        return self._dws

    def train_on_batch(self, ids_host: torch.Tensor, dense_host: Optional[torch.Tensor], label_host: torch.Tensor) -> float:
        B = ids_host.shape[0]
        self.ids_dev[:B].copy_(ids_host, non_blocking=True)
        if self.n_dense:
            self.dense_dev[:B].copy_(dense_host, non_blocking=True)
        self.label_dev[:B].copy_(label_host, non_blocking=True)
        self.train_step_on_device(self.ids_dev[:B], self.dense_dev[:B] if self.n_dense else None, self.label_dev[:B])
        self.loss_host.copy_(self.loss_sum, non_blocking=True)
# ... 81 lines not shown
```

handyrec_b200/kernels.py:

```python
from __future__ import annotations

import ctypes
from typing import List, Optional, Sequence, Tuple

import torch

from . import _lib
from ._lib import ACT, POOL, FieldDesc, OptParams, TableDesc, call

__all__ = [
    "init_uniform", "embedding_fwd", "embedding_bwd_dense", "seq_pool_fwd", "seq_pool_bwd", "LookupPlan",
    "fm_fwd", "fm_bwd", "dense_fwd", "dense_bwd_x", "dense_bwd_w", "act_bwd", "dice_fwd", "dice_bwd",
    "lau_fwd", "lau_pack_params", "sigmoid_bce", "adam_step", "sgd_step", "adam_step_multi", "sgd_step_multi",
    "adagrad_step", "adagrad_step_multi", "ftrl_step", "ftrl_step_multi", "metric_scratch_bytes", "metric_update",
]


_raw_stream = getattr(torch._C, "_cuda_getCurrentRawStream", None)


def _stream() -> ctypes.c_void_p:
    if _raw_stream is not None:
        return ctypes.c_void_p(_raw_stream(torch.cuda.current_device()))
    return ctypes.c_void_p(torch.cuda.current_stream().cuda_stream)
# ... 59 lines not shown
    _chk(ids, torch.int32, "ids")
    V, D = table.shape
    n = ids.numel()
    out = torch.empty(*ids.shape, D, device=table.device, dtype=torch.float32)
    mask = torch.empty(*ids.shape, D, device=table.device, dtype=torch.uint8) if mask_zero else None
    oob = torch.zeros(2, device=table.device, dtype=torch.int32) if check_ids else None
    call("hrb_embedding_fwd", _p(table), V, D, _p(ids), n, _p(out), _p(mask), _p(oob), _stream())
    if check_ids:
        _raise_if_oob(oob, "hrb_embedding_fwd")
    return out, (mask.view(torch.bool) if mask is not None else None)


def embedding_bwd_dense(ids: torch.Tensor, dout: torch.Tensor, vocab: int, table: Optional[torch.Tensor] = None, l2_scale: float = 0.0) -> torch.Tensor:
    _chk(ids, torch.int32, "ids")
    _chk(dout, torch.float32, "dout")
    D = dout.shape[-1]
    n = ids.numel()
    need = ctypes.c_size_t(0)
    call("hrb_embedding_bwd_dense_workspace", n, D, ctypes.byref(need))
    ws = torch.empty(need.value, device=dout.device, dtype=torch.uint8)
    dtable = torch.empty(vocab, D, device=dout.device, dtype=torch.float32)
    call("hrb_embedding_bwd_dense", _p(ids), n, _p(dout), vocab, D, _p(table), float(l2_scale), _p(dtable), _p(ws), need.value, _stream())
    return dtable


def _mask_u8(mask: torch.Tensor) -> torch.Tensor:
    if mask.dtype == torch.bool:
        mask = mask.view(torch.uint8)
    return _chk(mask, torch.uint8, "mask")


def seq_pool_fwd(x: torch.Tensor, mask: Optional[torch.Tensor], method: str) -> torch.Tensor:
    assert method in ["mean", "max", "sum"], "Pooling method should be `mean`, `max`, or `sum`"
    if mask is None:
        raise ValueError("Embedding layer should set `mask_zero` as True")
    _chk(x, torch.float32, "x")
    B, L, D = x.shape
    out = torch.empty(B, 1, D, device=x.device, dtype=torch.float32)
    call("hrb_seq_pool_fwd", _p(x), _p(_mask_u8(mask)), B, L, D, POOL[method], _p(out), _stream())
    return out


def seq_pool_bwd(x: torch.Tensor, mask: torch.Tensor, dout: torch.Tensor, method: str) -> torch.Tensor:
    _chk(x, torch.float32, "x")
    _chk(dout, torch.float32, "dout")
    B, L, D = x.shape
    dx = torch.empty_like(x)
    call("hrb_seq_pool_bwd", _p(x), _p(_mask_u8(mask)), _p(dout), B, L, D, POOL[method], _p(dx), _stream())
    return dx


class LookupPlan:

    def __init__(self, tables: Sequence[torch.Tensor], fields: Sequence[Tuple[int, int, str, int, int]],
                 adam_m: Optional[Sequence[torch.Tensor]] = None, adam_v: Optional[Sequence[torch.Tensor]] = None,
                 accum: Optional[Sequence[torch.Tensor]] = None, linear: Optional[Sequence[torch.Tensor]] = None):
        self.tables = [_chk(t, torch.float32, "table") for t in tables]
        if accum is not None:
            if adam_m is not None:
                raise ValueError("LookupPlan: pass either adam_m (Adam) or accum (Adagrad / Ftrl), not both")
            adam_m = accum
        if linear is not None:
            if adam_v is not None:
                raise ValueError("LookupPlan: pass either adam_v (Adam) or linear (Ftrl), not both")
            adam_v = linear
        self.adam_m = list(adam_m) if adam_m is not None else None
        self.adam_v = list(adam_v) if adam_v is not None else None
        self.fields = [tuple(f) for f in fields]
        self.n_fields = len(self.fields)
        self.device = self.tables[0].device
        td = (TableDesc * len(self.tables))()
        for i, t in enumerate(self.tables):
            td[i].weight = t.data_ptr()
            td[i].adam_m = self.adam_m[i].data_ptr() if self.adam_m is not None and self.adam_m[i] is not None else 0
            td[i].adam_v = self.adam_v[i].data_ptr() if self.adam_v is not None and self.adam_v[i] is not None else 0
            td[i].rows, td[i].dim = t.shape[0], t.shape[1]
        fd = (FieldDesc * self.n_fields)()
        self.ids_cols = 0
        self.out_cols = 0
        self.pos_cols = 0
        for i, (ti, L, pool, ids_col, out_col) in enumerate(self.fields):
            fd[i].table, fd[i].seq_len, fd[i].pool, fd[i].ids_col, fd[i].out_col = ti, L, POOL[pool], ids_col, out_col
            self.ids_cols = max(self.ids_cols, ids_col + L)
            self.out_cols = max(self.out_cols, out_col + self.tables[ti].shape[1])
            self.pos_cols += L
        self._h = ctypes.c_void_p(0)
        with torch.cuda.device(self.device):
            call("hrb_plan_create", td, len(self.tables), fd, self.n_fields, ctypes.byref(self._h))
        self._ws = None

    def set_dense_grads(self, grads: Sequence[Optional[torch.Tensor]]) -> None:
        assert len(grads) == len(self.tables)
        self._dense_grads = list(grads)
        arr = (ctypes.c_void_p * len(grads))(*[(g.data_ptr() if g is not None else None) for g in grads])
        call("hrb_plan_set_dense_grads", self._h, arr)

    def mark_rows(self, ids: torch.Tensor, touched: Sequence[Optional[torch.Tensor]]) -> None:
        assert len(touched) == len(self.tables)
        ids_ld = self._ids_ld(ids)
        for t in touched:
            if t is not None:
                _chk(t, torch.float32, "touched")
        arr = (ctypes.c_void_p * len(touched))(*[(t.data_ptr() if t is not None else None) for t in touched])
        call("hrb_plan_mark_rows", self._h, _p(ids), ids_ld, ids.shape[0], arr, _stream())

    def pad_flags(self, ids: torch.Tensor, flags: torch.Tensor) -> None:
        _chk(flags, torch.float32, "flags")
        call("hrb_plan_pad_flags", self._h, _p(ids), self._ids_ld(ids), ids.shape[0], _p(flags), _stream())

    def ftrl_pad_step(self, flags: torch.Tensor, op: OptParams) -> None:
        call("hrb_plan_ftrl_pad_step", self._h, _p(flags), ctypes.byref(op), _stream())

    def __del__(self):
        try:
            h = getattr(self, "_h", None)
            if h is not None and h.value:
                _lib.lib().hrb_plan_destroy(h)
                self._h = None
        except Exception:
            pass

    def _ids_ld(self, ids: torch.Tensor) -> int:
        _chk(ids, torch.int32, "ids", contiguous=False)
        return _row_major_2d(ids, "ids")

    def forward(self, ids: torch.Tensor, out: Optional[torch.Tensor] = None, want_inv_count: bool = False,
                check_ids: bool = False, fm: Optional[Tuple[torch.Tensor, torch.Tensor]] = None, want_fm_sum: bool = False):
        B = ids.shape[0]
        ids_ld = self._ids_ld(ids)
        if out is None:
            out = torch.empty(B, self.out_cols, device=self.device, dtype=torch.float32)
        out_ld = _row_major_2d(_chk(out, torch.float32, "out", contiguous=False), "out")
        inv = torch.empty(B, self.n_fields, device=self.device, dtype=torch.float32) if want_inv_count else None
        oob = torch.zeros(2, device=self.device, dtype=torch.int32) if check_ids else None
        res = {"out": out, "inv_count": inv}
        if fm is None:
            call("hrb_lookup_fwd", self._h, _p(ids), ids_ld, B, _p(out), out_ld, _p(inv), _p(oob), _stream())
        else:
            w, w0 = fm
            D = self.tables[0].shape[1]
            fm_out = torch.empty(B, device=self.device, dtype=torch.float32)
            fm_sum = torch.empty(B, D, device=self.device, dtype=torch.float32) if want_fm_sum else None
            call("hrb_lookup_fm_fwd", self._h, _p(ids), ids_ld, B, _p(out), out_ld, _p(inv), _p(w), _p(w0), _p(fm_out), _p(fm_sum), _p(oob), _stream())
            res["fm_out"], res["fm_sum"] = fm_out, fm_sum
        if check_ids:
            _raise_if_oob(oob, "hrb_lookup_fwd")
        return res

    def workspace_bytes(self, batch: int) -> int:
        need = ctypes.c_size_t(0)
        call("hrb_lookup_bwd_workspace", self._h, self.ids_cols, batch, ctypes.byref(need))
        return need.value

    def backward_update(self, ids: torch.Tensor, dout: torch.Tensor, opt: str = "sgd", lr: float = 0.01, l2_scale: float = 0.0,
                        beta1: float = 0.9, beta2: float = 0.999, eps: float = 1e-7, step: int = 1,
                        workspace: Optional[torch.Tensor] = None, autotune: bool = False, l1: float = 0.0, l2: float = 0.0,
                        lr_power: float = -0.5, l2_shrinkage: float = 0.0) -> None:
        B = ids.shape[0]
        ids_ld = self._ids_ld(ids)
        dout_ld = _row_major_2d(_chk(dout, torch.float32, "dout", contiguous=False), "dout")
        need = self.workspace_bytes(B)
        if workspace is None:
            if self._ws is None or self._ws.numel() < need:
                self._ws = torch.empty(need, device=self.device, dtype=torch.uint8)
            workspace = self._ws
        op = OptParams()
        op.opt = {"sgd": _lib.OPT_SGD, "adagrad": _lib.OPT_ADAGRAD, "ftrl": _lib.OPT_FTRL}.get(opt, _lib.OPT_ADAM_LAZY)
        op.lr, op.beta1, op.beta2, op.eps, op.l2_scale = lr, beta1, beta2, eps, l2_scale
        op.bias_corr1, op.bias_corr2 = 1.0 - beta1 ** step, 1.0 - beta2 ** step
        op.l1, op.l2, op.lr_power, op.l2_shrinkage = l1, l2, lr_power, l2_shrinkage
        trial = self._next_bwd_trial(B) if autotune else None
        if trial is not None:
            call("hrb_plan_set_bwd_algo", self._h, _lib.BWD_UNITS if trial == "units" else _lib.BWD_SORT)
            e0, e1 = torch.cuda.Event(enable_timing=True), torch.cuda.Event(enable_timing=True)
            e0.record()
        call("hrb_lookup_bwd_update", self._h, _p(ids), ids_ld, B, _p(dout), dout_ld, None, ctypes.byref(op), _p(workspace), workspace.numel(), _stream())
        if trial is not None:
            e1.record()
            e1.synchronize()
            self._finish_bwd_trial(trial, e0.elapsed_time(e1))

    _bwd_trial_log = None
    bwd_algo = "auto"

    def _next_bwd_trial(self, B: int) -> Optional[str]:
        if self.bwd_algo != "auto":
            return None
        if self._bwd_trial_log is None or self._bwd_trial_log["B"] != B:
            self._bwd_trial_log = {"B": B, "calls": 0, "units": [], "sort": []}
        log = self._bwd_trial_log
        log["calls"] += 1
        if log["calls"] <= 2:
            return None
        return "units" if len(log["units"]) <= len(log["sort"]) else "sort"

    def _finish_bwd_trial(self, trial: str, ms: float) -> None:
        log = self._bwd_trial_log
        log[trial].append(ms)
        if len(log["units"]) >= 2 and len(log["sort"]) >= 2:
            self.bwd_algo = "units" if min(log["units"]) <= min(log["sort"]) else "sort"
            self.bwd_algo_ms = {"units": min(log["units"]), "sort": min(log["sort"])}
            call("hrb_plan_set_bwd_algo", self._h, _lib.BWD_UNITS if self.bwd_algo == "units" else _lib.BWD_SORT)


def fm_fwd(x: torch.Tensor, w: torch.Tensor, w0: torch.Tensor, want_sum: bool = False):
    _chk(x, torch.float32, "x", contiguous=False)
    B, F, D = x.shape
    if x.stride(2) != 1 or x.stride(1) != D:
        raise ValueError("x must be a (B,F,D) view with contiguous (F,D) blocks")
    x_ld = x.stride(0) if B > 1 else F * D
    out = torch.empty(B, 1, device=x.device, dtype=torch.float32)
    s = torch.empty(B, D, device=x.device, dtype=torch.float32) if want_sum else None
    call("hrb_fm_fwd", _p(x), x_ld, B, F, D, _p(w), _p(w0), _p(out), _p(s), _stream())
    return (out, s) if want_sum else out


def fm_bwd(x: torch.Tensor, w: torch.Tensor, dout: torch.Tensor, dx: Optional[torch.Tensor] = None, accumulate: bool = False):
    B, F, D = x.shape
    x_ld = x.stride(0) if B > 1 else F * D
    if dx is None:
        dx = torch.empty(B, F, D, device=x.device, dtype=torch.float32)
        accumulate = False
    dx_ld = dx.stride(0) if B > 1 else F * D
    dwb = torch.empty(D + 1, device=x.device, dtype=torch.float32)
    call("hrb_fm_bwd", _p(x), x_ld, B, F, D, _p(w), _p(dout), _p(dx), dx_ld, int(accumulate), _p(dwb), _stream())
    return dx, dwb[:D].reshape(D, 1), dwb[D:]


def dense_fwd(x: torch.Tensor, w: torch.Tensor, bias: Optional[torch.Tensor], act: Optional[str] = None,
              out: Optional[torch.Tensor] = None, mode: int = _lib.GEMM_AUTO) -> torch.Tensor:
    M, K = x.shape
    N = w.shape[1]
    if out is None:
        out = torch.empty(M, N, device=x.device, dtype=torch.float32)
    call("hrb_dense_fwd", _p(x), _row_major_2d(x, "x"), _p(w), _row_major_2d(w, "w"), _p(bias), M, K, N, ACT[act], _p(out), _row_major_2d(out, "out"), mode, _stream())
    return out


def dense_bwd_x(dz: torch.Tensor, w: torch.Tensor, a_prev: Optional[torch.Tensor] = None, act_prev: Optional[str] = None,
                out: Optional[torch.Tensor] = None, mode: int = _lib.GEMM_AUTO) -> torch.Tensor:
    M, N = dz.shape
    K = w.shape[0]
    if out is None:
        out = torch.empty(M, K, device=dz.device, dtype=torch.float32)
    call("hrb_dense_bwd_x", _p(dz), _row_major_2d(dz, "dz"), _p(w), _row_major_2d(w, "w"), M, K, N, _p(a_prev),
         _row_major_2d(a_prev, "a_prev") if a_prev is not None else 0, ACT[act_prev], _p(out), _row_major_2d(out, "out"), mode, _stream())
    return out


_dense_ws = {}


def dense_bwd_w(x: torch.Tensor, dz: torch.Tensor, dw: Optional[torch.Tensor] = None, dbias: Optional[torch.Tensor] = None,
                want_bias: bool = True, mode: int = _lib.GEMM_AUTO):
    M, K = x.shape
    N = dz.shape[1]
    need = ctypes.c_size_t(0)
    call("hrb_dense_bwd_w_workspace", M, K, N, ctypes.byref(need))
    key = (x.device.index, _stream().value)
    ws = _dense_ws.get(key)
    if ws is None or ws.numel() < need.value:
        ws = torch.empty(need.value, device=x.device, dtype=torch.uint8)
        _dense_ws[key] = ws
    if dw is None:
        dw = torch.empty(K, N, device=x.device, dtype=torch.float32)
    if dbias is None and want_bias:
        dbias = torch.empty(N, device=x.device, dtype=torch.float32)
    call("hrb_dense_bwd_w", _p(x), _row_major_2d(x, "x"), _p(dz), _row_major_2d(dz, "dz"), M, K, N, _p(dw), _row_major_2d(dw, "dw"), _p(dbias), _p(ws), ws.numel(), mode, _stream())
    return dw, dbias


def act_bwd(y: torch.Tensor, dy: torch.Tensor, act: Optional[str]) -> torch.Tensor:
    dz = torch.empty_like(dy)
    call("hrb_act_bwd", _p(y.contiguous()), _p(dy.contiguous()), dy.numel(), ACT[act], _p(dz), _stream())
    return dz


def dice_fwd(x: torch.Tensor, alpha: torch.Tensor, mean: torch.Tensor, var: torch.Tensor, training: bool, eps: float = 1e-9):
    units = x.shape[-1]
    rows = x.numel() // units
    y = torch.empty_like(x)
    call("hrb_dice_fwd", _p(_chk(x, torch.float32, "x")), rows, units, _p(alpha), _p(mean), _p(var), eps, int(training), _p(y), _stream())
    return y


def dice_bwd(x: torch.Tensor, dy: torch.Tensor, alpha: torch.Tensor, mean: torch.Tensor, var: torch.Tensor, training: bool, eps: float = 1e-9):
    units = x.shape[-1]
    rows = x.numel() // units
    dx = torch.empty_like(x)
    dalpha = torch.empty(units, device=x.device, dtype=torch.float32)
    scratch = torch.empty(2 * units, device=x.device, dtype=torch.float32)
    call("hrb_dice_bwd", _p(x), _p(_chk(dy, torch.float32, "dy")), rows, units, _p(alpha), _p(mean), _p(var), eps, int(training), _p(dx), _p(dalpha), _p(scratch), _stream())
    return dx, dalpha


def lau_pack_params(Ws: Sequence[torch.Tensor], bs: Sequence[torch.Tensor], dice: Optional[Sequence[Tuple[torch.Tensor, torch.Tensor, torch.Tensor]]] = None) -> torch.Tensor:
    chunks: List[torch.Tensor] = []
    n = len(Ws)
    total = 0
    for i, (W, b) in enumerate(zip(Ws, bs)):
        parts = [W.reshape(-1), b.reshape(-1)]
        if dice is not None and i != n - 1:
            parts += [t.reshape(-1) for t in dice[i]]
        for p in parts:
            chunks.append(p.to(torch.float32))
            total += p.numel()
        pad = (-total) % 4
        if pad:
            chunks.append(torch.zeros(pad, device=Ws[0].device, dtype=torch.float32))
            total += pad
    return torch.cat(chunks).contiguous()


def lau_fwd(table: torch.Tensor, query_ids: torch.Tensor, key_ids: torch.Tensor, params: torch.Tensor, layer_out: Sequence[int],
            act: Optional[str], want_pooled: bool = True):
    V, D = table.shape
    B, T = key_ids.shape
    score = torch.empty(B, 1, T, device=table.device, dtype=torch.float32)
    pooled = torch.empty(B, 1, D, device=table.device, dtype=torch.float32) if want_pooled else None
    lo = (ctypes.c_int32 * len(layer_out))(*layer_out)
    call("hrb_lau_fwd", _p(table), V, D, _p(_chk(query_ids, torch.int32, "query_ids")), _p(_chk(key_ids, torch.int32, "key_ids")), B, T,
         _p(params), lo, len(layer_out), ACT[act], _p(score), _p(pooled), _stream())
    return score, pooled


def sigmoid_bce(dnn_logit: torch.Tensor, fm_logit: Optional[torch.Tensor], label: torch.Tensor, grad_scale: float,
                prob: Optional[torch.Tensor] = None, dlogit: Optional[torch.Tensor] = None, loss_sum: Optional[torch.Tensor] = None):
    B = dnn_logit.numel()
    call("hrb_sigmoid_bce", _p(dnn_logit), _p(fm_logit), _p(label), B, grad_scale, _p(prob), _p(dlogit), _p(loss_sum), _stream())


def adam_step(param, grad, m, v, lr, beta1=0.9, beta2=0.999, eps=1e-7, step=1, l2_scale=0.0):
    call("hrb_adam_step", _p(param), _p(grad), _p(m), _p(v), param.numel(), lr, beta1, beta2, eps, 1.0 - beta1 ** step, 1.0 - beta2 ** step, l2_scale, _stream())
# ... 181 lines not shown
```

handyrec_b200/sharded.py:

```python
from __future__ import annotations

import ctypes
from typing import List, Optional, Sequence, Tuple

import torch

from . import _lib
from . import kernels as K
from ._lib import call
from .engine import DeepFMEngine


def shard_rows(vocab: int, rank: int, n_ranks: int) -> int:
    return max(1, (vocab - rank + n_ranks - 1) // n_ranks)


def key_base_table(vocabs: Sequence[int], n_ranks: int) -> torch.Tensor:
    kb = torch.zeros(n_ranks, len(vocabs), dtype=torch.int64)
    for r in range(n_ranks):
        acc = 0
        for t, v in enumerate(vocabs):
            kb[r, t] = acc
            acc += shard_rows(v, r, n_ranks)
    return kb
# ... 83 lines not shown
    def all_to_all_v(self, send: torch.Tensor, send_counts: List[int], recv_counts: List[int]) -> torch.Tensor:
        recv = torch.empty((sum(recv_counts),) + tuple(send.shape[1:]), device=send.device, dtype=send.dtype)
        self.dist.all_to_all_single(recv, send, output_split_sizes=recv_counts, input_split_sizes=send_counts, group=self.group)
        return recv

    def all_to_all_v_start(self, send: torch.Tensor, send_counts: List[int], recv_counts: List[int]):
        recv = torch.empty((sum(recv_counts),) + tuple(send.shape[1:]), device=send.device, dtype=send.dtype)
        work = self.dist.all_to_all_single(recv, send, output_split_sizes=recv_counts, input_split_sizes=send_counts, group=self.group, async_op=True)
        return recv, work.wait

    def all_gather_equal(self, send: torch.Tensor) -> torch.Tensor:
        out = torch.empty((self.N,) + tuple(send.shape), device=send.device, dtype=send.dtype)
        self.dist.all_gather_into_tensor(out, send.contiguous(), group=self.group)
        return out

    def all_reduce_sum(self, t: torch.Tensor) -> None:
        self.dist.all_reduce(t, group=self.group)

    def alloc_receive_buffers(self, rows: int, dim: int, device) -> Optional["ReceiveBuffers"]:
        if self.dist.get_backend(self.group) != "nccl":
            return None
        import torch.distributed._symmetric_memory as symm_mem

        g_elems = (rows * dim + 63) // 64 * 64
        arena = symm_mem.empty((g_elems + rows,), dtype=torch.float32, device=device)
        hdl = symm_mem.rendezvous(arena, group=self.group if self.group is not None else self.dist.group.WORLD)
        grads = arena[: rows * dim].view(rows, dim)
        keys = arena[g_elems : g_elems + rows].view(torch.int32)
        base = [int(p) for p in hdl.buffer_ptrs]
        return ReceiveBuffers(arena, hdl, grads, keys, base, [b + g_elems * 4 for b in base])

    _dense_group = None

    def all_reduce_dense(self, t: torch.Tensor) -> None:
        if self._dense_group is None:
            nccl = self.dist.get_backend(self.group) == "nccl"
            ranks = None if self.group is None else self.dist.get_process_group_ranks(self.group)
            self._dense_group = self.dist.new_group(ranks=ranks) if nccl else self.group
        self.dist.all_reduce(t, group=self._dense_group)

    def alloc_tables(self, vocabs: Sequence[int], dim: int, device, replicate_max_rows: int = 0) -> Tuple[List[torch.Tensor], Optional[List[List[int]]]]:
        rep = [v <= replicate_max_rows for v in vocabs]
        rows = [v if r else shard_rows(v, self.rank, self.N) for v, r in zip(vocabs, rep)]
        if self.dist.get_backend(self.group) != "nccl":
            return [torch.zeros(r, dim) for r in rows], None
        import torch.distributed._symmetric_memory as symm_mem

        offs, off = [], 0
        for v, r in zip(vocabs, rep):
            offs.append(off)
            if not r:
                off += (shard_rows(v, 0, self.N) * dim + 63) // 64 * 64
        arena = symm_mem.empty((max(off, 64),), dtype=torch.float32, device=device)
        hdl = symm_mem.rendezvous(arena, group=self.group if self.group is not None else self.dist.group.WORLD)
        self._arena, self._arena_hdl = arena, hdl
        tables = [torch.zeros(n, dim, device=device) if r else arena[o : o + n * dim].view(n, dim) for o, n, r in zip(offs, rows, rep)]
        peer_ptrs = [[0 if r else int(hdl.buffer_ptrs[rk]) + o * 4 for o, r in zip(offs, rep)] for rk in range(self.N)]
        return tables, peer_ptrs


class RowExchange:

    def __init__(self, provider, comm):
        self.p, self.comm = provider, comm
        self.N = comm.N
        self.rx: Optional[ReceiveBuffers] = None

    def route_async(self, ids: torch.Tensor) -> None:
        self.perm, self.send_keys, counts = self.p.route(ids)
        self._counts_dev = counts
        if self.rx is not None:
            self._count_matrix_dev = self.comm.all_gather_equal(counts[: self.N])
        else:
            self._recv_counts_dev = self.comm.all_to_all_equal(counts[: self.N].contiguous())
        self._routed = False
        self._route_done = None
        if self.perm.is_cuda:
            self._route_done = torch.cuda.Event()
            self._route_done.record()

    def finish_route(self) -> None:
        if self._routed:
            return
        if getattr(self, "_route_done", None) is not None:
            torch.cuda.current_stream().wait_event(self._route_done)
        if self.rx is not None:
            C = self._count_matrix_dev.tolist()
            self.send_counts, self.recv_counts, self.dst_off = exchange_offsets(C, self.comm.rank)
            self.n_send, self.n_recv = sum(self.send_counts), sum(self.recv_counts)
            if self.n_recv > self.rx.keys.shape[0]:
                raise RuntimeError(f"gradient exchange: {self.n_recv} rows for this owner exceed the receive buffer ({self.rx.keys.shape[0]})")
            self.recv_keys = None
            self._routed = True
            return
        both = torch.cat([self._counts_dev[: self.N], self._recv_counts_dev]).tolist()
        self.send_counts, self.recv_counts = [int(x) for x in both[: self.N]], [int(x) for x in both[self.N :]]
        self.n_send, self.n_recv = sum(self.send_counts), sum(self.recv_counts)
        self.recv_keys = self.comm.all_to_all_v(self.send_keys[: self.n_send], self.send_counts, self.recv_counts)
        self._routed = True

    def forward(self, ids: torch.Tensor, out: torch.Tensor) -> None:
        if self.rx is not None:
            raise RuntimeError("the all-to-all forward needs the keys exchanged: do not attach receive buffers in this mode")
        self.route_async(ids)
        self.finish_route()
        rows = self.p.rows_by_key(self.recv_keys, self.n_recv)
        got = self.comm.all_to_all_v(rows, self.recv_counts, self.send_counts)
        self.p.scatter_rows(ids, self.perm, self.n_send, got, out)

    def backward_start(self, ids: torch.Tensor, dout: torch.Tensor) -> None:
        self.finish_route()
        if getattr(self, "_route_done", None) is not None:
            torch.cuda.current_stream().wait_event(self._route_done)
        if self.rx is not None:
            self.p.scatter_grads_to_owners(ids, self.perm, self.send_keys, dout, self.send_counts, self.dst_off, self.rx)
            self._grad_send = self._grad_recv = self._grad_wait = None
            return
        self._grad_send = self.p.gather_grads(ids, self.perm, self.n_send, dout)
        start = getattr(self.comm, "all_to_all_v_start", None)
        if start is not None:
            self._grad_recv, self._grad_wait = start(self._grad_send, self.send_counts, self.recv_counts)
        else:
            self._grad_recv, self._grad_wait = self.comm.all_to_all_v(self._grad_send, self.send_counts, self.recv_counts), None

    def backward_finish(self, op, mark=None) -> None:
        if self.rx is not None:
            self.rx.barrier(0)
            if mark is not None:
                mark("grad_rows_p2p_scatter")
            self.p.keyed_update(self.rx.keys, self.rx.grads, self.n_recv, op)
            if mark is not None:
                mark("keyed_update")
            return
        if self._grad_wait is not None:
            self._grad_wait()
        if mark is not None:
            mark("grad_rows_all_to_all")
        if self._grad_recv.is_cuda:
            cur = torch.cuda.current_stream()
            self._grad_recv.record_stream(cur)
            self._grad_send.record_stream(cur)
            self.recv_keys.record_stream(cur)
        self.p.keyed_update(self.recv_keys, self._grad_recv, self.n_recv, op)
        self._grad_send = self._grad_recv = self._grad_wait = None
        if mark is not None:
            mark("keyed_update")

    def backward_update(self, ids: torch.Tensor, dout: torch.Tensor, op, mark=None) -> None:
        self.backward_start(ids, dout)
        self.backward_finish(op, mark)


class ShardedDeepFMEngine(DeepFMEngine):

    def __init__(self, tables, vocabs, fields, n_dense, comm, peer_ptrs=None, replicate_max_rows: int = 0, replicated=None,
                 p2p_grad_exchange: bool = True, **kw):
        if replicated is None:
            replicated = [t for t, v in enumerate(vocabs) if v <= replicate_max_rows]
        self.replicated = sorted(set(int(t) for t in replicated))
        n_sharded = len(tables) - len(self.replicated)
        pooled = any(pool not in (None, "none") for ti, L, pool in fields if ti not in self.replicated)
        self._n_pad_flags = 2 * n_sharded if kw.get("optimizer") == "ftrl" and pooled else 0
        for t in self.replicated:
            if tables[t].shape[0] != vocabs[t]:
                raise ValueError(f"replicated table {t} must be a full copy ({vocabs[t]} rows), got {tables[t].shape[0]}")
        super().__init__(tables, fields, n_dense, dense_update_tables=self.replicated, **kw)
        self.comm = comm
        self.world = comm.N
        n_t = len(self.tables)
        self.sharded = [t for t in range(n_t) if t not in self.replicated]
        def sub_plan(tabs, with_moments):
            remap = {t: i for i, t in enumerate(tabs)}
            flds = [(remap[f[0]],) + tuple(f[1:]) for f in self.plan_fields if f[0] in remap]
            if not flds:
                return None
            m = [self.adam_m[t] for t in tabs] if (with_moments and self.adam_m is not None) else None
            v = [self.adam_v[t] for t in tabs] if (with_moments and self.adam_v is not None) else None
            acc = [self.accum[t] for t in tabs] if (with_moments and self.accum is not None) else None
            lin = [self.linear[t] for t in tabs] if (with_moments and self.linear is not None) else None
            return K.LookupPlan([self.tables[t] for t in tabs], flds, m, v, accum=acc, linear=lin)

        if self.replicated:
            self.plan_shard = sub_plan(self.sharded, True)
            self.plan_rep = sub_plan(self.replicated, False)
            if self.plan_rep is not None:
                self.plan_rep.set_dense_grads([self.table_grads[t] for t in self.replicated])
                self._ws_rep = torch.empty(self.plan_rep.workspace_bytes(self.B), device=self.dev, dtype=torch.uint8)
        else:
            self.plan_shard, self.plan_rep = self.plan, None
        self._pad_flags = self.grads[-self._n_pad_flags :] if self._n_pad_flags else None
        self.exchange = None
        if self.plan_shard is not None:
            self.provider = CudaShardProvider(self.plan_shard, [vocabs[t] for t in self.sharded], comm.N, self.B)
            self.exchange = RowExchange(self.provider, comm)
        self.grad_scale_div = comm.N
        self.overlap_embedding_bwd = True
        self.peer_lookup = False
        self._rep_done = None
        self._barrier_buf = torch.zeros(1, device=self.dev)
        plain = all(f[1] == 1 and f[2] in ("none", None) for f in fields)
        if self.exchange is None and plain:
            self.peer_lookup = True
        elif peer_ptrs is not None and plain:
            ptrs = (ctypes.c_void_p * (comm.N * n_t))(
                *[(None if t in self.replicated else int(peer_ptrs[r][t])) for r in range(comm.N) for t in range(n_t)])
            full = (ctypes.c_int64 * n_t)(*[int(v) for v in vocabs])
            call("hrb_plan_set_peers", self.plan._h, comm.N, ptrs, full)
            self.peer_lookup = True
            if p2p_grad_exchange and hasattr(comm, "alloc_receive_buffers"):
                self.exchange.rx = comm.alloc_receive_buffers(comm.N * self.B * self.plan_shard.pos_cols, self.D, self.dev)

    _fwd_training = False

    def forward(self, ids, dense, training: bool = False):
        self._fwd_training = training
        return super().forward(ids, dense, training)

    def _lookup_fm_forward(self, ids, B, st):
        if self.peer_lookup:
            super()._lookup_fm_forward(ids, B, st)
            if self.exchange is not None and self._fwd_training:
                main = torch.cuda.current_stream()
                if self._side is None:
                    self._side = torch.cuda.Stream()
                if self._marks is None:
                    self._side.wait_stream(main)
                    with torch.cuda.stream(self._side):
                        self.exchange.route_async(ids)
                else:
                    self.exchange.route_async(ids)
                    self._mark("route_ids")
            return
        if self.exchange is not None:
            self.exchange.forward(ids, self.X0)
        if self.plan_rep is not None:
            call("hrb_lookup_fwd", self.plan_rep._h, K._p(ids), ids.stride(0), B, K._p(self.X0), self.K0p, None, None, st)
        self._mark("sharded_lookup_fwd")
        emb = self.X0[:, self.nd_pad :]
        call("hrb_fm_fwd", K._p(emb), self.K0p, B, self.F, self.D, K._p(self.fm_w), K._p(self.fm_w0), K._p(self.fm_out), K._p(self.fm_sum), st)
        self._mark("fm_fwd")

    def _pre_embedding_backward(self):
        if self.peer_lookup and self.exchange is not None:
            self.exchange.finish_route()
            if self._timeline is not None:
                self._mark("route_keys_all_to_all")

    _side2 = None

    def _embedding_backward(self, ids, B, st, op):
        cur = torch.cuda.current_stream()
        own_stream = False
        if self.exchange is not None:
            self.exchange.backward_start(ids, self.dX0)
            own_stream = self._marks is None and self.plan_rep is not None and self.dX0.is_cuda
            if own_stream:
                if self._side2 is None:
                    self._side2 = torch.cuda.Stream()
                self._side2.wait_stream(cur)
                with torch.cuda.stream(self._side2):
                    self._finish_sharded(op)
        if self.plan_rep is None and self._pad_flags is not None:
            self._zero_table_grads()
            self.plan_shard.pad_flags(ids, self._pad_flags)
            self._rep_done = torch.cuda.Event()
            self._rep_done.record()
        if self.plan_rep is not None:
            self._zero_table_grads()
            self._mark_touched(self.plan_rep, ids, self.replicated)
            if self._pad_flags is not None:
                self.plan_shard.pad_flags(ids, self._pad_flags)
            call("hrb_lookup_bwd_update", self.plan_rep._h, K._p(ids), ids.stride(0), B, K._p(self.dX0), self.K0p, None, ctypes.byref(op),
                 K._p(self._ws_rep), self._ws_rep.numel(), K._stream())
            self._rep_done = torch.cuda.Event()
            self._rep_done.record()
            self._mark("replicated_embedding_bwd")
        if self.exchange is not None:
            if own_stream:
                cur.wait_stream(self._side2)
            else:
                self._finish_sharded(op)
            self._mark("sharded_embedding_bwd_update")

    def _finish_sharded(self, op):
        self.exchange.backward_finish(op, mark=self._mark if self._timeline is not None else None)
        if self.peer_lookup:
            if self.exchange.rx is not None:
                self.exchange.rx.barrier(1)
            else:
                self.comm.all_reduce_sum(self._barrier_buf)

    def _sync_dense_grads(self):
        if self._rep_done is not None:
            torch.cuda.current_stream().wait_event(self._rep_done)
            self._rep_done = None
        getattr(self.comm, "all_reduce_dense", self.comm.all_reduce_sum)(self.grads)
        self._mark("dense_allreduce")
        if self._pad_flags is not None and self.comm.rank == 0:
            self.plan_shard.ftrl_pad_step(self._pad_flags, self._op)
```

include/hrb200.h:

```cpp
#ifndef HRB200_H_
#define HRB200_H_

#include <stddef.h>
#include <stdint.h>

#ifdef __cplusplus
extern "C" {
#endif

#define HRB_ABI_VERSION 1

typedef enum hrb_status {
  HRB_OK = 0,
  HRB_BAD_ARG = 1,
  HRB_UNSUPPORTED = 2,
  HRB_CUDA_ERROR = 3,
  HRB_WORKSPACE = 4
} hrb_status;

typedef enum hrb_pool { HRB_POOL_NONE = 0, HRB_POOL_MEAN = 1, HRB_POOL_SUM = 2, HRB_POOL_MAX = 3 } hrb_pool;

typedef enum hrb_act {
  HRB_ACT_LINEAR = 0,
  HRB_ACT_RELU = 1,
  HRB_ACT_SIGMOID = 2,
  HRB_ACT_TANH = 3,
  HRB_ACT_DICE = 4
} hrb_act;

int hrb_abi_version(void);
const char* hrb_status_str(int status);
const char* hrb_last_error(void);
int hrb_launch_count(int64_t* count);

int hrb_init_uniform(float* table, int64_t rows, int32_t dim, uint32_t seed, float lo, float hi,
                     int64_t row_start, int64_t row_step, void* stream);

int hrb_embedding_fwd(const float* table, int64_t vocab, int32_t dim, const int32_t* ids, int64_t n_ids,
                      float* out, uint8_t* mask, int32_t* oob, void* stream);

int hrb_embedding_bwd_dense_workspace(int64_t n_ids, int32_t dim, size_t* bytes);
int hrb_embedding_bwd_dense(const int32_t* ids, int64_t n_ids, const float* dout, int64_t vocab, int32_t dim,
                            const float* table, float l2_scale, float* dtable, void* workspace,
                            size_t workspace_bytes, void* stream);

int hrb_seq_pool_fwd(const float* x, const uint8_t* mask, int64_t batch, int32_t seq_len, int32_t dim,
                     int32_t method, float* out, void* stream);
int hrb_seq_pool_bwd(const float* x, const uint8_t* mask, const float* dout, int64_t batch, int32_t seq_len,
                     int32_t dim, int32_t method, float* dx, void* stream);

typedef struct hrb_table_desc {
  float* weight;
  float* adam_m;
  float* adam_v;
  int64_t rows;
  int32_t dim;
  int32_t pad_;
} hrb_table_desc;

typedef struct hrb_field_desc {
  int32_t table;
  int32_t seq_len;
  int32_t pool;
  int32_t ids_col;
  int32_t out_col;
  int32_t pad_;
} hrb_field_desc;

typedef struct hrb_plan hrb_plan;

int hrb_plan_create(const hrb_table_desc* tables_host, int32_t n_tables, const hrb_field_desc* fields_host,
                    int32_t n_fields, hrb_plan** plan);
int hrb_plan_destroy(hrb_plan* plan);

int hrb_lookup_fwd(const hrb_plan* plan, const int32_t* ids, int64_t ids_ld, int64_t batch, float* out,
                   int64_t out_ld, float* inv_count, int32_t* oob, void* stream);

int hrb_lookup_fm_fwd(const hrb_plan* plan, const int32_t* ids, int64_t ids_ld, int64_t batch, float* out,
                      int64_t out_ld, float* inv_count, const float* fm_w, const float* fm_w0, float* fm_out,
                      float* fm_sum, int32_t* oob, void* stream);

typedef enum hrb_opt { HRB_OPT_SGD = 0, HRB_OPT_ADAM_LAZY = 1, HRB_OPT_ADAGRAD = 2, HRB_OPT_FTRL = 3 } hrb_opt;
typedef struct hrb_opt_params {
  int32_t opt;
  float lr, beta1, beta2, eps, l2_scale;
  float bias_corr1, bias_corr2;
  float l1, l2, lr_power, l2_shrinkage;
} hrb_opt_params;
int hrb_lookup_bwd_workspace(const hrb_plan* plan, int64_t ids_ld, int64_t batch, size_t* bytes);
int hrb_lookup_bwd_update(const hrb_plan* plan, const int32_t* ids, int64_t ids_ld, int64_t batch,
                          const float* dout, int64_t dout_ld, const float* inv_count,
                          const hrb_opt_params* opt_host, void* workspace, size_t workspace_bytes,
                          void* stream);

typedef enum hrb_bwd_algo { HRB_BWD_AUTO = 0, HRB_BWD_UNITS = 1, HRB_BWD_SORT = 2 } hrb_bwd_algo;
int hrb_plan_set_bwd_algo(hrb_plan* plan, int32_t algo);

int hrb_plan_set_dense_grads(hrb_plan* plan, float* const* grads_host);

int hrb_plan_mark_rows(const hrb_plan* plan, const int32_t* ids, int64_t ids_ld, int64_t batch, float* const* touched_host,
                       void* stream);
int hrb_plan_pad_flags(const hrb_plan* plan, const int32_t* ids, int64_t ids_ld, int64_t batch, float* flags, void* stream);
int hrb_plan_ftrl_pad_step(const hrb_plan* plan, const float* flags, const hrb_opt_params* opt_host, void* stream);

int hrb_fm_fwd(const float* x, int64_t x_ld, int64_t batch, int32_t fields, int32_t dim, const float* w,
               const float* w0, float* out, float* fm_sum, void* stream);
int hrb_fm_bwd(const float* x, int64_t x_ld, int64_t batch, int32_t fields, int32_t dim, const float* w,
               const float* dout, float* dx, int64_t dx_ld, int32_t accumulate, float* dw_dw0, void* stream);

typedef enum hrb_gemm_mode { HRB_GEMM_AUTO = 0, HRB_GEMM_FP32 = 1, HRB_GEMM_3XTF32 = 2 } hrb_gemm_mode;
int hrb_dense_fwd(const float* x, int64_t ldx, const float* w, int64_t ldw, const float* bias, int64_t M,
                  int32_t K, int32_t N, int32_t act, float* y, int64_t ldy, int32_t mode, void* stream);
int hrb_dense_bwd_x(const float* dz, int64_t lddz, const float* w, int64_t ldw, int64_t M, int32_t K,
                    int32_t N, const float* a_prev, int64_t lda_prev, int32_t act_prev, float* dx,
                    int64_t lddx, int32_t mode, void* stream);
int hrb_dense_bwd_w_workspace(int64_t M, int32_t K, int32_t N, size_t* bytes);
int hrb_dense_bwd_w(const float* x, int64_t ldx, const float* dz, int64_t lddz, int64_t M, int32_t K,
                    int32_t N, float* dw, int64_t lddw, float* dbias, void* workspace, size_t workspace_bytes,
                    int32_t mode, void* stream);
int hrb_transpose(const float* src, int64_t rows, int32_t cols, int64_t lds, float* dst, int64_t ldd, void* stream);
int hrb_dense_fwd_t(const float* x, int64_t ldx, const float* wt, int64_t ldwt, const float* bias, int64_t M, int32_t K,
                    int32_t N, int32_t act, float* y, int64_t ldy, float* yt, int64_t ldyt, uint32_t* relu_mask, void* stream);
int hrb_dense_bwd_x_t(const float* dz, int64_t lddz, const float* w, int64_t ldw, int64_t M, int32_t K, int32_t N,
                      const float* a_prev, int64_t lda_prev, int32_t act_prev, const uint32_t* relu_mask, float* dx, int64_t lddx,
                      float* dxt, int64_t lddxt, void* stream);
int hrb_dense_bwd_w_t_workspace(int64_t M, int32_t K, int32_t N, size_t* bytes);
int hrb_dense_bwd_w_t(const float* xt, int64_t ldxt, const float* dzt, int64_t lddzt, const float* dz, int64_t lddz, int64_t M,
                      int32_t K, int32_t N, float* dw, int64_t lddw, float* dbias, void* workspace, size_t workspace_bytes,
                      void* stream);
int hrb_dense_bwd_w_xn(const float* x, int64_t ldx, const float* dzt, int64_t lddzt, int64_t M, int32_t K, int32_t N, float* dw,
                       int64_t lddw, float* dbias, void* workspace, size_t workspace_bytes, void* stream);

int hrb_dense1_fwd(const float* x, int64_t ldx, const float* w, const float* bias, int64_t M, int32_t K, float* y, void* stream);
int hrb_dense1_bwd_workspace(int64_t M, int32_t K, size_t* bytes);
int hrb_dense1_bwd(const float* x, int64_t ldx, const float* w, const float* dy, int64_t M, int32_t K, int32_t act_prev,
                   float* dz_prev, int64_t lddz, float* dz_prev_t, int64_t lddzt, float* dw, float* dbias, void* workspace,
                   size_t workspace_bytes, void* stream);

int hrb_act_bwd(const float* y, const float* dy, int64_t n, int32_t act, float* dz, void* stream);

int hrb_dice_fwd(const float* x, int64_t rows, int32_t units, const float* alpha, float* mean, float* var,
                 float eps, int32_t training, float* y, void* stream);
int hrb_dice_bwd(const float* x, const float* dy, int64_t rows, int32_t units, const float* alpha,
                 const float* mean, const float* var, float eps, int32_t training, float* dx, float* dalpha,
                 float* scratch , void* stream);

int hrb_batchnorm_fwd(const float* x, int64_t rows, int32_t units, const float* gamma, const float* beta, float* mean,
                      float* var, float eps, int32_t training, float* y, void* stream);
int hrb_batchnorm_bwd(const float* x, const float* dy, int64_t rows, int32_t units, const float* gamma, const float* mean,
                      const float* var, float eps, int32_t training, float* dx, float* dgamma, float* dbeta,
                      float* scratch , void* stream);
int hrb_dropout(const float* x, int64_t n, float rate, uint32_t seed, float* y, void* stream);

int hrb_lau_fwd(const float* table, int64_t vocab, int32_t dim, const int32_t* query_ids,
                const int32_t* key_ids, int64_t batch, int32_t seq_len, const float* params,
                const int32_t* layer_out_host, int32_t n_layers, int32_t act, float* score, float* pooled,
                void* stream);

int hrb_att_input_fwd(const float* q, const float* k, int64_t batch, int32_t T, int32_t D, float* out, void* stream);
int hrb_att_input_bwd(const float* q, const float* k, const float* g, int64_t batch, int32_t T, int32_t D, float* dq,
                      float* dk, void* stream);
int hrb_mask_scores(const float* s, const uint8_t* mask, int64_t n, float* out, void* stream);
int hrb_att_pool_fwd(const float* s, const float* k, int64_t batch, int32_t T, int32_t D, float* out, void* stream);
int hrb_att_pool_bwd(const float* s, const float* k, const float* dout, int64_t batch, int32_t T, int32_t D, float* ds,
                     float* dk, void* stream);

int hrb_lau_split_weights(const float* w, int64_t ldw, int32_t dim, int32_t units, float* wq, float* wp, float* wpt, void* stream);
int hrb_lau_merge_wgrads(const float* dwq, const float* dwp, int32_t dim, int32_t units, float* dw, int64_t ldw, void* stream);
int hrb_lau_pack_fwd(const float* q, const float* k, int64_t batch, int32_t T, int32_t dim, float* out, void* stream);
int hrb_lau_pack_bwd(const float* q, const float* k, const float* da, int64_t batch, int32_t T, int32_t dim, int32_t accumulate_dq,
                     float* dq, float* dk, void* stream);
int hrb_group_sum(const float* x, int64_t ldx, int64_t groups, int32_t group_rows, int32_t n, float* out, void* stream);
int hrb_dense_fwd_t_grouped(const float* x, int64_t ldx, const float* wt, int64_t ldwt, const float* group_bias, int64_t ldgb,
                            int32_t group_rows, int64_t M, int32_t K, int32_t N, int32_t act, float* y, int64_t ldy, void* stream);

int hrb_sigmoid_bce(const float* dnn_logit, const float* fm_logit, const float* label, int64_t batch,
                    float grad_scale, float* prob, float* dlogit, float* loss_sum, void* stream);

int hrb_clipped_bce(const float* prob, const float* label, int64_t n, float eps, float grad_scale, float* dprob,
                    float* loss_sum, void* stream);

int hrb_sampled_softmax(const float* true_logit, const float* sampled_logit, int64_t ld, const int32_t* labels,
                        const int32_t* sampled, int64_t batch, int32_t num_sampled, const float* true_expected,
                        const float* sampled_expected, float num_tries, int64_t range_max, int32_t remove_accidental_hits,
                        const float* gout, float* loss, float* d_true_logit, float* d_sampled_logit, void* stream);
int hrb_rowdot(const float* a, int64_t lda, const float* b, int64_t ldb, int64_t M, int32_t K, float* out, void* stream);
int hrb_rowscale(const float* x, int64_t ldx, const float* s, int64_t M, int32_t K, float* out, int64_t ldo, void* stream);
int hrb_l2_normalize_fwd(const float* x, int64_t n, float eps, float* y, float* stat, float* scratch, void* stream);
int hrb_l2_normalize_bwd(const float* y, const float* dy, int64_t n, const float* stat, float* dx, float* scratch, void* stream);

int hrb_topk_init(float* best_val, int32_t* best_idx, int64_t queries, int32_t k, void* stream);
int hrb_topk_merge(const float* scores, int64_t ld, int64_t queries, int32_t n_cols, int64_t col_base, int32_t k, float* best_val,
                   int32_t* best_idx, void* stream);

#define HRB_METRIC_MAX_THRESHOLDS 8192
typedef enum hrb_metric_kind {
  HRB_METRIC_TP = 0,
  HRB_METRIC_FP = 1,
  HRB_METRIC_TN = 2,
  HRB_METRIC_FN = 3,
  HRB_METRIC_CORRECT = 4,
  HRB_METRIC_COUNT = 5
} hrb_metric_kind;
int hrb_metric_scratch_bytes(int32_t n_thr, size_t* bytes);
int hrb_metric_update(const float* prob, const float* label, int64_t n, const float* thresholds, int32_t n_thr,
                      const int32_t* var_kind, const int32_t* var_thr, int32_t n_vars, float* vars, void* scratch, int32_t* flags,
                      void* stream);

int hrb_pack_dense(const void* src, int32_t src_is_int32, int64_t src_ld, int64_t batch, int32_t n, int32_t n_pad,
                   float* dst, int64_t dst_ld, void* stream);

int hrb_host_pack_i32(const void* const* cols_host, const int32_t* dtype_host, const int64_t* width_host, const int64_t* ld_host,
                      int32_t n_cols, int64_t row_start, int64_t rows, int32_t* dst_host, int64_t dst_ld, int32_t n_threads);
int hrb_host_pack_f32(const void* const* cols_host, const int32_t* dtype_host, const int64_t* width_host, const int64_t* ld_host,
                      int32_t n_cols, int64_t row_start, int64_t rows, float* dst_host, int64_t dst_ld, int32_t n_threads);

int hrb_host_pack_set_writeback(int32_t on);

int hrb_adam_step(float* param, const float* grad, float* m, float* v, int64_t n, float lr, float beta1,
                  float beta2, float eps, float bias_corr1, float bias_corr2, float l2_scale, void* stream);
int hrb_sgd_step(float* param, const float* grad, int64_t n, float lr, float l2_scale, void* stream);
int hrb_adagrad_step(float* param, const float* grad, float* acc, int64_t n, float lr, float eps, float l2_scale, void* stream);
int hrb_ftrl_step(float* param, const float* grad, float* acc, float* lin, int64_t n, float lr, float l1, float l2, float lr_power,
                  float l2_shrinkage, float l2_scale, const float* row_touched, int32_t dim, void* stream);
#define HRB_MULTI_MAX 32
int hrb_adam_step_multi(int32_t count, float* const* param_host, const float* const* grad_host, float* const* m_host,
                        float* const* v_host, const int64_t* n_host, const float* l2_scale_host, float lr, float beta1,
                        float beta2, float eps, float bias_corr1, float bias_corr2, void* stream);
int hrb_sgd_step_multi(int32_t count, float* const* param_host, const float* const* grad_host, const int64_t* n_host,
                       const float* l2_scale_host, float lr, void* stream);
int hrb_adagrad_step_multi(int32_t count, float* const* param_host, const float* const* grad_host, float* const* acc_host,
                           const int64_t* n_host, const float* l2_scale_host, float lr, float eps, void* stream);
int hrb_ftrl_step_multi(int32_t count, float* const* param_host, const float* const* grad_host, float* const* acc_host,
                        float* const* lin_host, const int64_t* n_host, const float* l2_scale_host, float lr, float l1, float l2,
                        float lr_power, float l2_shrinkage, void* stream);


int hrb_enable_peer_access(int32_t peer_device);
int hrb_plan_set_peers(hrb_plan* plan, int32_t n_ranks, const void* const* peer_tables_host, const int64_t* full_rows_host);
int hrb_plan_set_full_rows(hrb_plan* plan, const int64_t* full_rows_host);
int hrb_route_workspace(const hrb_plan* plan, int64_t batch, size_t* bytes);
int hrb_route_ids(const hrb_plan* plan, const int32_t* ids, int64_t ids_ld, int64_t batch, int32_t n_ranks,
                  const uint32_t* key_base, uint32_t* perm, uint32_t* send_keys, int64_t* counts, void* workspace,
                  size_t workspace_bytes, void* stream);
int hrb_rows_by_key(const hrb_plan* plan, const uint32_t* keys, int64_t n, float* out, void* stream);
int hrb_scatter_rows(const hrb_plan* plan, const int32_t* ids, int64_t ids_ld, int64_t batch, const uint32_t* perm, int64_t n,
// ... 17 lines not shown
```

Baseline: 53.75 million.

## Split embedding backward into early partition on side stream and later apply

Moves the id partitioning (count, scan, scatter) of the embedding backward onto a separate stream that starts at the top of the training step, so it overlaps with the forward and dense backward. The apply/update kernel then waits on an event. The prep transpose kernel is fused into the count kernel, and the separate scan kernel is folded in through a last-block-done atomic counter, cutting two launches. This adds cross-stream synchronization and a global done counter that must reset correctly, and it is disabled for the sharded engine.

```diff
diff --git a/handyrec_b200/csrc/embedding_bwd.cu b/handyrec_b200/csrc/embedding_bwd.cu
--- a/handyrec_b200/csrc/embedding_bwd.cu
+++ b/handyrec_b200/csrc/embedding_bwd.cu
@@ -22,7 +22,6 @@
 constexpr int UB_WARPS = UB_THREADS / 32;
 constexpr int UB_HELPERS = 4;
 constexpr int UB_TILE = 4096;
-constexpr int SPLIT_ROUNDS = UB_TILE / UB_WARPS / 32;
 constexpr uint32_t UB_INVALID = 0xFFFFFFFFu;
 constexpr uint32_t UB_NONE = 0xFFFFFFFEu;
 constexpr int UB_SLICE_TARGET = 4096;
@@ -31,40 +30,6 @@
 constexpr int UB_APPLY = 2;
 
 static inline size_t ub_align(size_t x, size_t a = 256) { return (x + a - 1) / a * a; }
-
-__global__ void __launch_bounds__(256) bwd_prep_kernel(const FieldDev* __restrict__ fields, const int32_t* __restrict__ pos_field,
-                                                      int32_t pos_cols, const int32_t* __restrict__ ids, int64_t ids_ld, int64_t batch,
-                                                      int64_t ldT, uint32_t* __restrict__ idsT) {
-  __shared__ uint32_t tile[32][33];
-  const int tx = threadIdx.x & 31, ty = threadIdx.x >> 5;
-  const int64_t b0 = (int64_t)blockIdx.x * 32;
-  const int c0 = blockIdx.y * 32;
-  const int c = c0 + tx;
-  int ids_col = 0, pool = 0;
-  int64_t rows = 0;
-  if (c < pos_cols) {
-    const FieldDev& f = fields[pos_field[c]];
-    ids_col = f.ids_col + (c - f.pos_col);
-    pool = f.pool;
-    rows = f.rows;
-  }
-  for (int r = ty; r < 32; r += 8) {
-    const int64_t b = b0 + r;
-    uint32_t v = UB_INVALID;
-    if (b < batch && c < pos_cols) {
-      const int32_t id = ids[b * ids_ld + ids_col];
-      const bool valid = (pool == HRB_POOL_NONE || id != 0) && id >= 0 && (int64_t)id < rows;
-      if (valid) v = (uint32_t)id;
-    }
-    tile[r][tx] = v;
-  }
-  __syncthreads();
-  for (int r = ty; r < 32; r += 8) {
-    const int cc = c0 + r;
-    const int64_t b = b0 + tx;
-    if (cc < pos_cols && b < ldT) idsT[(int64_t)cc * ldT + b] = tile[tx][r];
-  }
-}
 
 __global__ void __launch_bounds__(256) bwd_scale_kernel(const FieldDev* __restrict__ fields, int32_t n_fields,
                                                        const int32_t* __restrict__ ids, int64_t ids_ld, int64_t batch,
@@ -88,94 +53,116 @@
   }
 }
 
+constexpr int SPLIT_MAX_REGS = 96;
+constexpr int SPLIT_MAX_SMEM = 24 * 1024;
+constexpr int SPLIT_WARP_SAMPLES = UB_TILE / UB_WARPS;
+static_assert(UB_THREADS == UB_MAX_BINS, "the table scan gives every thread of the last CTA one bin");
+
 struct SplitArgs {
   const TableSplitDev* splits;
   const TileDev* tiles;
-  const uint32_t* idsT;
-  int64_t ldT;
+  const FieldDev* fields;
+  const int32_t* pos_field;
+  const int32_t* ids;
+  int64_t ids_ld, batch;
+  uint32_t* idsT;
   uint32_t* tile_cnt;
   uint32_t* list_cnt;
   uint32_t* list_off;
   uint32_t* ent_row;
   uint32_t* ent_pos;
+  uint32_t* done;
 };
 
-template <bool SCATTER>
-__global__ void __launch_bounds__(UB_THREADS) split_kernel(SplitArgs a) {
-  __shared__ uint32_t wcnt[UB_WARPS][UB_MAX_BINS];
-  const int tid = threadIdx.x, lane = tid & 31, w = tid >> 5;
-  const TileDev tile = a.tiles[blockIdx.x];
-  const TableSplitDev ts = a.splits[tile.table];
-  for (int i = tid; i < UB_WARPS * UB_MAX_BINS; i += UB_THREADS) (&wcnt[0][0])[i] = 0;
-  __syncthreads();
-  const uint32_t* colp = a.idsT + (int64_t)tile.pos_col * a.ldT;
-  const int64_t b0 = (int64_t)tile.chunk * UB_TILE + w * (UB_TILE / UB_WARPS);
-  uint32_t packed[SPLIT_ROUNDS];
-  uint32_t idv[SPLIT_ROUNDS];
-#pragma unroll
-  for (int k = 0; k < SPLIT_ROUNDS; ++k) {
-    const int64_t b = b0 + k * 32 + lane;
-    idv[k] = b < a.ldT ? __ldg(colp + b) : UB_INVALID;
-  }
-#pragma unroll
-  for (int k = 0; k < SPLIT_ROUNDS; ++k) {
-    const uint32_t id = idv[k];
-    const uint32_t bin = id == UB_INVALID ? UB_INVALID : id >> ts.shift;
+struct SplitSmem {
+  uint32_t id[UB_TILE];
+  uint32_t wcnt[UB_WARPS][UB_MAX_BINS];
+};
+static_assert(sizeof(SplitSmem) <= SPLIT_MAX_SMEM, "level-1 shared memory budget");
+
+__host__ __device__ inline int64_t split_ldT(int64_t batch) { return (batch + UB_TILE - 1) / UB_TILE * UB_TILE; }
+
+__device__ __forceinline__ void split_gather_tile(SplitSmem& s, const SplitArgs& a, const TileDev& tile) {
+  const int tid = threadIdx.x;
+  for (int i = tid; i < UB_WARPS * UB_MAX_BINS; i += UB_THREADS) (&s.wcnt[0][0])[i] = 0;
+  const FieldDev& f = a.fields[a.pos_field[tile.pos_col]];
+  const int32_t pool = f.pool;
+  const int64_t rows = f.rows;
+  const int32_t* col = a.ids + f.ids_col + (tile.pos_col - f.pos_col);
+  const int64_t b0 = (int64_t)tile.chunk * UB_TILE;
+  constexpr int K = UB_TILE / UB_THREADS;
+  int32_t v[K];
+#pragma unroll
+  for (int k = 0; k < K; ++k) {
+    const int64_t b = b0 + k * UB_THREADS + tid;
+    v[k] = b < a.batch ? __ldg(col + b * a.ids_ld) : -1;
+  }
+#pragma unroll
+  for (int k = 0; k < K; ++k) {
+    const int32_t id = v[k];
+    const bool valid = (pool == HRB_POOL_NONE || id != 0) && id >= 0 && (int64_t)id < rows;
+    s.id[k * UB_THREADS + tid] = valid ? (uint32_t)id : UB_INVALID;
+    a.idsT[tile.pos_col * split_ldT(a.batch) + b0 + k * UB_THREADS + tid] = valid ? (uint32_t)id : UB_INVALID;
+  }
+}
+
+template <bool COUNT>
+__device__ __forceinline__ void split_walk(SplitSmem& s, const SplitArgs& a, const TileDev& tile, int shift) {
+  const int lane = threadIdx.x & 31, w = threadIdx.x >> 5;
+  const uint32_t mask = (1u << shift) - 1u;
+  const int64_t b0 = (int64_t)tile.chunk * UB_TILE + w * SPLIT_WARP_SAMPLES;
+  for (int k = 0; k < SPLIT_WARP_SAMPLES / 32; ++k) {
+    const uint32_t id = s.id[w * SPLIT_WARP_SAMPLES + k * 32 + lane];
+    const uint32_t bin = id == UB_INVALID ? UB_INVALID : id >> shift;
     const uint32_t peers = __match_any_sync(0xffffffffu, bin);
     const int leader = __ffs(peers) - 1;
     uint32_t base = 0;
     if (bin != UB_INVALID && lane == leader) {
-      base = wcnt[w][bin];
-      wcnt[w][bin] = base + __popc(peers);
-    }
-    if (SCATTER) {
+      base = s.wcnt[w][bin];
+      s.wcnt[w][bin] = base + __popc(peers);
+    }
+    if (!COUNT) {
       base = __shfl_sync(0xffffffffu, base, leader);
-      packed[k] = bin == UB_INVALID ? UB_INVALID : (bin << 16) | (base + __popc(peers & ((1u << lane) - 1u)));
+      if (bin != UB_INVALID) {
+        const uint32_t dst = base + __popc(peers & ((1u << lane) - 1u));
+        a.ent_row[dst] = id & mask;
+        a.ent_pos[dst] = ((uint32_t)tile.col_local << 24) | (uint32_t)(b0 + k * 32 + lane);
+      }
     }
     __syncwarp();
   }
+}
+
+__global__ void __launch_bounds__(UB_THREADS) split_count_kernel(SplitArgs a) {
+  __shared__ SplitSmem s;
+  const int tid = threadIdx.x;
+  const TileDev tile = a.tiles[blockIdx.x];
+  const TableSplitDev ts = a.splits[tile.table];
+  split_gather_tile(s, a, tile);
+  __syncthreads();
+  split_walk<true>(s, a, tile, ts.shift);
   __syncthreads();
   uint32_t* tc = a.tile_cnt + (size_t)blockIdx.x * UB_MAX_BINS;
-  if (!SCATTER) {
-    for (int u = tid; u < ts.n_bins; u += UB_THREADS) {
-      uint32_t t = 0;
-#pragma unroll
-      for (int ww = 0; ww < UB_WARPS; ++ww) t += wcnt[ww][u];
-      tc[u] = t;
-    }
-    return;
-  }
   for (int u = tid; u < ts.n_bins; u += UB_THREADS) {
-    uint32_t run = tc[u];
-#pragma unroll
-    for (int ww = 0; ww < UB_WARPS; ++ww) {
-      const uint32_t t = wcnt[ww][u];
-      wcnt[ww][u] = run;
-      run += t;
-    }
-  }
-  __syncthreads();
-  const uint32_t mask = (1u << ts.shift) - 1u;
-#pragma unroll
-  for (int k = 0; k < SPLIT_ROUNDS; ++k) {
-    if (packed[k] == UB_INVALID) continue;
-    const int64_t b = b0 + k * 32 + lane;
-    const uint32_t id = idv[k];
-    const uint32_t dst = wcnt[w][packed[k] >> 16] + (packed[k] & 0xFFFFu);
-    a.ent_row[dst] = id & mask;
-    a.ent_pos[dst] = ((uint32_t)tile.col_local << 24) | (uint32_t)b;
-  }
-}
-
-__global__ void __launch_bounds__(UB_MAX_BINS) split_scan_kernel(SplitArgs a) {
-  __shared__ uint32_t tot[UB_MAX_BINS];
-  const TableSplitDev ts = a.splits[blockIdx.x];
-  const int u = threadIdx.x;
+    uint32_t t = 0;
+#pragma unroll
+    for (int ww = 0; ww < UB_WARPS; ++ww) t += s.wcnt[ww][u];
+    tc[u] = t;
+  }
+  __threadfence();
+  __syncthreads();
+  if (tid == 0) s.id[0] = atomicAdd(a.done + tile.table, 1u) == (uint32_t)ts.n_tiles - 1;
+  __syncthreads();
+  if (!s.id[0]) return;
+  __threadfence();
+  if (tid == 0) a.done[tile.table] = 0;
+  uint32_t* tot = s.wcnt[0];
+  const int u = tid;
   uint32_t run = 0;
   if (u < ts.n_bins) {
     for (int t = 0; t < ts.n_tiles; ++t) {
       uint32_t* p = a.tile_cnt + (size_t)(ts.first_tile + t) * UB_MAX_BINS + u;
-      const uint32_t c = *p;
+      const uint32_t c = __ldcg(p);
       *p = run;
       run += c;
     }
@@ -194,6 +181,31 @@
     a.list_off[ts.first_list + u] = base;
     for (int t = 0; t < ts.n_tiles; ++t) a.tile_cnt[(size_t)(ts.first_tile + t) * UB_MAX_BINS + u] += base;
   }
+}
+
+__global__ void __launch_bounds__(UB_THREADS) split_scatter_kernel(SplitArgs a) {
+  __shared__ SplitSmem s;
+  const int tid = threadIdx.x;
+  const TileDev tile = a.tiles[blockIdx.x];
+  const TableSplitDev ts = a.splits[tile.table];
+  for (int i = tid; i < UB_WARPS * UB_MAX_BINS; i += UB_THREADS) (&s.wcnt[0][0])[i] = 0;
+  const uint4* src = reinterpret_cast<const uint4*>(a.idsT + tile.pos_col * split_ldT(a.batch) + (int64_t)tile.chunk * UB_TILE);
+  for (int i = tid; i < UB_TILE / 4; i += UB_THREADS) reinterpret_cast<uint4*>(s.id)[i] = __ldcg(src + i);
+  __syncthreads();
+  split_walk<true>(s, a, tile, ts.shift);
+  __syncthreads();
+  const uint32_t* tc = a.tile_cnt + (size_t)blockIdx.x * UB_MAX_BINS;
+  for (int u = tid; u < ts.n_bins; u += UB_THREADS) {
+    uint32_t run = tc[u];
+#pragma unroll
+    for (int ww = 0; ww < UB_WARPS; ++ww) {
+      const uint32_t t = s.wcnt[ww][u];
+      s.wcnt[ww][u] = run;
+      run += t;
+    }
+  }
+  __syncthreads();
+  split_walk<false>(s, a, tile, ts.shift);
 }
 
 struct UnitArgs {
@@ -693,8 +705,6 @@
   int64_t expect;
 };
 
-static inline int64_t unit_ldT(int64_t batch) { return (batch + 15) / 16 * 16; }
-
 static int build_units(const hrb_plan* plan, int64_t batch) {
   UnitSet& us = plan->units;
   if (us.batch == batch) return HRB_OK;
@@ -706,7 +716,7 @@
   std::vector<TableSplitDev> splits(plan->n_tables);
   std::vector<TileDev> tiles;
   int32_t n_partials = 0, n_lists = 0;
-  const int64_t n_chunks = (unit_ldT(batch) + UB_TILE - 1) / UB_TILE;
+  const int64_t n_chunks = (batch + UB_TILE - 1) / UB_TILE;
   std::vector<int32_t> col_pos;
   for (int t = 0; t < plan->n_tables; ++t)
     for (int f = 0; f < plan->n_fields; ++f) {
@@ -794,8 +804,10 @@
   us.d_blob = nullptr;
   const size_t sz_u = ub_align(sizeof(UnitDev) * (ud.size() + 1)), sz_g = ub_align(sizeof(SliceGroupDev) * (gd.size() + 1));
   const size_t sz_s = ub_align(sizeof(TableSplitDev) * (splits.size() + 1)), sz_t = ub_align(sizeof(TileDev) * (tiles.size() + 1));
-  HRB_CUDA(cudaMalloc(&us.d_blob, sz_u + sz_g + sz_s + sz_t));
+  const size_t sz_d = ub_align(sizeof(uint32_t) * (splits.size() + 1));
+  HRB_CUDA(cudaMalloc(&us.d_blob, sz_u + sz_g + sz_s + sz_t + sz_d));
   char* d = (char*)us.d_blob;
+  HRB_CUDA(cudaMemset(d + sz_u + sz_g + sz_s + sz_t, 0, sz_d));
   if (!ud.empty()) HRB_CUDA(cudaMemcpy(d, ud.data(), sizeof(UnitDev) * ud.size(), cudaMemcpyHostToDevice));
   if (!gd.empty()) HRB_CUDA(cudaMemcpy(d + sz_u, gd.data(), sizeof(SliceGroupDev) * gd.size(), cudaMemcpyHostToDevice));
   HRB_CUDA(cudaMemcpy(d + sz_u + sz_g, splits.data(), sizeof(TableSplitDev) * splits.size(), cudaMemcpyHostToDevice));
@@ -804,6 +816,7 @@
   us.d_groups = (SliceGroupDev*)(d + sz_u);
   us.d_splits = (TableSplitDev*)(d + sz_u + sz_g);
   us.d_tiles = (TileDev*)(d + sz_u + sz_g + sz_s);
+  us.d_done = (uint32_t*)(d + sz_u + sz_g + sz_s + sz_t);
   us.n_units = (int32_t)ud.size();
   us.n_groups = (int32_t)gd.size();
   us.n_partials = n_partials;
@@ -832,7 +845,7 @@
     return o;
   };
   const size_t n = (size_t)batch * plan->pos_cols;
-  w.idsT = take((size_t)plan->pos_cols * unit_ldT(batch) * 4);
+  w.idsT = take((size_t)plan->pos_cols * split_ldT(batch) * 4);
   w.scale = take((size_t)batch * plan->n_fields * 4 + 4);
   w.partials = take((size_t)(us.n_partials + 1) * UB_PARTIAL_LD * 4);
   w.ent_row = take(n * 4 + 4);
@@ -872,51 +885,58 @@
   return HRB_OK;
 }
 
-int run_unit_update(const hrb_plan* plan, const int32_t* ids, int64_t ids_ld, int64_t batch, const float* dout, int64_t dout_ld,
-                    const hrb_opt_params& opt, void* workspace, size_t workspace_bytes, cudaStream_t st) {
+int run_unit_partition(const hrb_plan* plan, const int32_t* ids, int64_t ids_ld, int64_t batch, void* workspace, size_t workspace_bytes,
+                       const char* who, cudaStream_t st) {
   std::lock_guard<std::mutex> lock(plan->unit_mu);
   int rc = build_units(plan, batch);
   if (rc != HRB_OK) return rc;
   const UnitSet& us = plan->units;
   if (!us.ok) return fail(HRB_UNSUPPORTED, "embedding backward: unit path not available for this plan / batch");
   const UnitWs ws = carve_unit_ws(plan, batch);
-  if (ws.total > workspace_bytes) return fail(HRB_WORKSPACE, "hrb_lookup_bwd_update: workspace %zu < required %zu bytes", workspace_bytes, ws.total);
+  if (ws.total > workspace_bytes) return fail(HRB_WORKSPACE, "%s: workspace %zu < required %zu bytes", who, workspace_bytes, ws.total);
   char* base = (char*)workspace;
-  const int64_t ldT = unit_ldT(batch);
-  uint32_t* idsT = (uint32_t*)(base + ws.idsT);
-  float* scale = (float*)(base + ws.scale);
-  dim3 pg((unsigned)((ldT + 31) / 32), (unsigned)((plan->pos_cols + 31) / 32));
-  bwd_prep_kernel<<<pg, 256, 0, st>>>(plan->d_fields, plan->d_pos_field, plan->pos_cols, ids, ids_ld, batch, ldT, idsT);
-  HRB_LAUNCH_CHECK();
   if (plan->has_mean) {
     int64_t blocks = (batch * plan->n_fields + 255) / 256;
     const int64_t cap = (int64_t)sm_count() * 8;
     if (blocks > cap) blocks = cap;
-    bwd_scale_kernel<<<(unsigned)blocks, 256, 0, st>>>(plan->d_fields, plan->n_fields, ids, ids_ld, batch, scale);
+    bwd_scale_kernel<<<(unsigned)blocks, 256, 0, st>>>(plan->d_fields, plan->n_fields, ids, ids_ld, batch, (float*)(base + ws.scale));
     HRB_LAUNCH_CHECK();
   }
-  SplitArgs sa{us.d_splits, us.d_tiles, idsT, ldT, (uint32_t*)(base + ws.tile_cnt), (uint32_t*)(base + ws.list_cnt),
-               (uint32_t*)(base + ws.list_off), (uint32_t*)(base + ws.ent_row), (uint32_t*)(base + ws.ent_pos)};
   if (us.n_tiles > 0) {
-    split_kernel<false><<<us.n_tiles, UB_THREADS, 0, st>>>(sa);
+    SplitArgs sa{us.d_splits, us.d_tiles, plan->d_fields, plan->d_pos_field, ids, ids_ld, batch, (uint32_t*)(base + ws.idsT),
+                 (uint32_t*)(base + ws.tile_cnt),
+                 (uint32_t*)(base + ws.list_cnt), (uint32_t*)(base + ws.list_off), (uint32_t*)(base + ws.ent_row),
+                 (uint32_t*)(base + ws.ent_pos), us.d_done};
+    split_count_kernel<<<us.n_tiles, UB_THREADS, 0, st>>>(sa);
     HRB_LAUNCH_CHECK();
-    split_scan_kernel<<<plan->n_tables, UB_MAX_BINS, 0, st>>>(sa);
+    split_scatter_kernel<<<us.n_tiles, UB_THREADS, 0, st>>>(sa);
     HRB_LAUNCH_CHECK();
-    split_kernel<true><<<us.n_tiles, UB_THREADS, 0, st>>>(sa);
-    HRB_LAUNCH_CHECK();
-  }
+  }
+  return HRB_OK;
+}
+
+int run_unit_apply(const hrb_plan* plan, int64_t batch, const float* dout, int64_t dout_ld, const hrb_opt_params& opt, void* workspace,
+                   size_t workspace_bytes, const char* who, cudaStream_t st) {
+  std::lock_guard<std::mutex> lock(plan->unit_mu);
+  int rc = build_units(plan, batch);
+  if (rc != HRB_OK) return rc;
+  const UnitSet& us = plan->units;
+  if (!us.ok) return fail(HRB_UNSUPPORTED, "embedding backward: unit path not available for this plan / batch");
+  const UnitWs ws = carve_unit_ws(plan, batch);
+  if (ws.total > workspace_bytes) return fail(HRB_WORKSPACE, "%s: workspace %zu < required %zu bytes", who, workspace_bytes, ws.total);
+  char* base = (char*)workspace;
   UnitArgs a{};
   a.units = us.d_units;
   a.tables = plan->d_tables;
   a.cols = plan->d_cols;
   a.col_start = plan->d_col_start;
-  a.list_cnt = sa.list_cnt;
-  a.list_off = sa.list_off;
-  a.ent_row = sa.ent_row;
-  a.ent_pos = sa.ent_pos;
+  a.list_cnt = (const uint32_t*)(base + ws.list_cnt);
+  a.list_off = (const uint32_t*)(base + ws.list_off);
+  a.ent_row = (const uint32_t*)(base + ws.ent_row);
+  a.ent_pos = (const uint32_t*)(base + ws.ent_pos);
   a.dout = dout;
   a.dout_ld = dout_ld;
-  a.scale = plan->has_mean ? scale : nullptr;
+  a.scale = plan->has_mean ? (const float*)(base + ws.scale) : nullptr;
   a.n_fields = plan->n_fields;
   a.opt = opt;
   a.lr_t = opt.opt == HRB_OPT_ADAM_LAZY ? opt.lr * sqrtf(opt.bias_corr2) / opt.bias_corr1 : 0.f;
diff --git a/handyrec_b200/csrc/lookup.cu b/handyrec_b200/csrc/lookup.cu
--- a/handyrec_b200/csrc/lookup.cu
+++ b/handyrec_b200/csrc/lookup.cu
@@ -1317,64 +1317,127 @@
   return HRB_OK;
 }
 
+static int bwd_check(const hrb_plan* plan, const int32_t* ids, const float* dout, int64_t dout_ld, const hrb_opt_params* opt_host,
+                     const void* workspace, int64_t batch, const char* who) {
+  HRB_REQUIRE(plan && ids && dout && opt_host && workspace && batch >= 0, "%s: null/negative argument", who);
+  HRB_REQUIRE(aligned16(dout) && dout_ld % 4 == 0, "%s: dout must be 16-byte aligned, dout_ld %% 4 == 0", who);
+  if (plan->has_max)
+    return fail(HRB_UNSUPPORTED, "%s: max-pooled fields go through hrb_seq_pool_bwd + hrb_embedding_bwd_dense", who);
+  const hrb_opt_params opt = load_opt(opt_host);
+  HRB_REQUIRE(opt.opt == HRB_OPT_SGD || opt.opt == HRB_OPT_ADAM_LAZY || opt.opt == HRB_OPT_ADAGRAD || opt.opt == HRB_OPT_FTRL,
+              "%s: unknown optimiser %d", who, opt.opt);
+  if (opt.opt == HRB_OPT_ADAM_LAZY)
+    for (const auto& t : plan->tdev_host)
+      HRB_REQUIRE(t.grad || (t.m && t.v), "%s: lazy Adam needs adam_m/adam_v for every table", who);
+  if (opt.opt == HRB_OPT_ADAGRAD)
+    for (const auto& t : plan->tdev_host)
+      HRB_REQUIRE(t.grad || t.m, "%s: Adagrad needs an accumulator (adam_m) for every row-updated table", who);
+  if (opt.opt == HRB_OPT_FTRL) {
+    int rc = ftrl_tables_ok(plan, who);
+    if (rc != HRB_OK) return rc;
+  }
+  if (plan->max_dim / 4 > 256) return fail(HRB_UNSUPPORTED, "%s: dim %d too large", who, plan->max_dim);
+  HRB_REQUIRE(batch * plan->pos_cols < 0x7FFFFFFFll, "%s: batch*sum(seq_len) exceeds 2^31-1", who);
+  return HRB_OK;
+}
+
+static size_t bwd_body_bytes(const hrb_plan* plan, size_t workspace_bytes, bool pad) {
+  const size_t fb = pad ? pad_flag_bytes(plan) : 0;
+  return (workspace_bytes - fb) / 256 * 256;
+}
+
+static int bwd_partition(const hrb_plan* plan, const int32_t* ids, int64_t ids_ld, int64_t batch, void* workspace,
+                         size_t workspace_bytes, bool pad, const char* who, cudaStream_t st) {
+  if (batch == 0) return HRB_OK;
+  if (pad) {
+    const size_t fb = pad_flag_bytes(plan);
+    if (workspace_bytes < fb) return fail(HRB_WORKSPACE, "%s: workspace %zu < %zu bytes of padding flags", who, workspace_bytes, fb);
+    float* flags = (float*)((char*)workspace + bwd_body_bytes(plan, workspace_bytes, true));
+    int rc = launch_pad_flags(plan, ids, ids_ld, batch, flags, st);
+    if (rc != HRB_OK) return rc;
+  }
+  const bool units = plan->bwd_algo != HRB_BWD_SORT && unit_path_supported(plan, batch);
+  if (units) {
+    int rc = run_unit_partition(plan, ids, ids_ld, batch, workspace, bwd_body_bytes(plan, workspace_bytes, pad), who, st);
+    if (rc != HRB_OK) return rc;
+  }
+  std::lock_guard<std::mutex> lock(plan->unit_mu);
+  plan->bwd_part = hrb_plan::BwdPartition{batch, workspace, workspace_bytes, units, pad};
+  return HRB_OK;
+}
+
 static int run_plan_sorted_update(const hrb_plan* plan, const int32_t* ids, int64_t ids_ld, int64_t batch, const float* dout,
-                                  int64_t dout_ld, const hrb_opt_params& opt, void* workspace, size_t workspace_bytes, cudaStream_t st);
+                                  int64_t dout_ld, const hrb_opt_params& opt, void* workspace, size_t workspace_bytes, const char* who,
+                                  cudaStream_t st);
+
+static int bwd_apply(const hrb_plan* plan, const int32_t* ids, int64_t ids_ld, int64_t batch, const float* dout, int64_t dout_ld,
+                     const hrb_opt_params* opt_host, void* workspace, size_t workspace_bytes, const char* who, cudaStream_t st) {
+  if (batch == 0) return HRB_OK;
+  hrb_plan::BwdPartition part;
+  {
+    std::lock_guard<std::mutex> lock(plan->unit_mu);
+    part = plan->bwd_part;
+    plan->bwd_part = hrb_plan::BwdPartition{};
+  }
+  if (part.batch != batch || part.workspace != workspace || part.workspace_bytes != workspace_bytes)
+    return fail(HRB_BAD_ARG, "%s: no hrb_lookup_bwd_partition of this plan, batch and workspace precedes it", who);
+  const hrb_opt_params opt = load_opt(opt_host);
+  const bool pad = opt.opt == HRB_OPT_FTRL && has_pooled(plan);
+  if (pad && !part.pad) return fail(HRB_BAD_ARG, "%s: Ftrl with pooled fields needs the padding flags of hrb_lookup_bwd_partition", who);
+  const bool units = plan->bwd_algo != HRB_BWD_SORT && unit_path_supported(plan, batch);
+  if (units != part.units) return fail(HRB_BAD_ARG, "%s: the backward algorithm changed since hrb_lookup_bwd_partition", who);
+  const size_t body = bwd_body_bytes(plan, workspace_bytes, part.pad);
+  int rc = units ? run_unit_apply(plan, batch, dout, dout_ld, opt, workspace, body, who, st)
+                 : run_plan_sorted_update(plan, ids, ids_ld, batch, dout, dout_ld, opt, workspace, body, who, st);
+  if (rc != HRB_OK || !pad) return rc;
+  return launch_ftrl_pad(plan, (const float*)((char*)workspace + body), opt, st);
+}
+
+HRB_API int hrb_lookup_bwd_partition(const hrb_plan* plan, const int32_t* ids, int64_t ids_ld, int64_t batch, void* workspace,
+                                     size_t workspace_bytes, void* stream) {
+  HRB_REQUIRE(plan && ids && workspace && batch >= 0, "hrb_lookup_bwd_partition: null/negative argument");
+  if (plan->has_max)
+    return fail(HRB_UNSUPPORTED, "hrb_lookup_bwd_partition: max-pooled fields go through hrb_seq_pool_bwd + hrb_embedding_bwd_dense");
+  HRB_REQUIRE(batch * plan->pos_cols < 0x7FFFFFFFll, "hrb_lookup_bwd_partition: batch*sum(seq_len) exceeds 2^31-1");
+  return bwd_partition(plan, ids, ids_ld, batch, workspace, workspace_bytes, has_pooled(plan), "hrb_lookup_bwd_partition",
+                       (cudaStream_t)stream);
+}
+
+HRB_API int hrb_lookup_bwd_apply(const hrb_plan* plan, const int32_t* ids, int64_t ids_ld, int64_t batch, const float* dout,
+                                 int64_t dout_ld, const float* inv_count, const hrb_opt_params* opt_host, void* workspace,
+                                 size_t workspace_bytes, void* stream) {
+  (void)inv_count;
+  int rc = bwd_check(plan, ids, dout, dout_ld, opt_host, workspace, batch, "hrb_lookup_bwd_apply");
+  if (rc != HRB_OK) return rc;
+  return bwd_apply(plan, ids, ids_ld, batch, dout, dout_ld, opt_host, workspace, workspace_bytes, "hrb_lookup_bwd_apply",
+                   (cudaStream_t)stream);
+}
 
 HRB_API int hrb_lookup_bwd_update(const hrb_plan* plan, const int32_t* ids, int64_t ids_ld, int64_t batch,
                                   const float* dout, int64_t dout_ld, const float* inv_count,
                                   const hrb_opt_params* opt_host, void* workspace, size_t workspace_bytes,
                                   void* stream) {
   (void)inv_count;
-  HRB_REQUIRE(plan && ids && dout && opt_host && workspace && batch >= 0, "hrb_lookup_bwd_update: null/negative argument");
-  HRB_REQUIRE(aligned16(dout) && dout_ld % 4 == 0, "hrb_lookup_bwd_update: dout must be 16-byte aligned, dout_ld %% 4 == 0");
-  if (plan->has_max)
-    return fail(HRB_UNSUPPORTED, "hrb_lookup_bwd_update: max-pooled fields go through hrb_seq_pool_bwd + hrb_embedding_bwd_dense");
-  const hrb_opt_params opt = load_opt(opt_host);
-  HRB_REQUIRE(opt.opt == HRB_OPT_SGD || opt.opt == HRB_OPT_ADAM_LAZY || opt.opt == HRB_OPT_ADAGRAD || opt.opt == HRB_OPT_FTRL,
-              "hrb_lookup_bwd_update: unknown optimiser %d", opt.opt);
-  if (opt.opt == HRB_OPT_ADAM_LAZY)
-    for (const auto& t : plan->tdev_host)
-      HRB_REQUIRE(t.grad || (t.m && t.v), "hrb_lookup_bwd_update: lazy Adam needs adam_m/adam_v for every table");
-  if (opt.opt == HRB_OPT_ADAGRAD)
-    for (const auto& t : plan->tdev_host)
-      HRB_REQUIRE(t.grad || t.m, "hrb_lookup_bwd_update: Adagrad needs an accumulator (adam_m) for every row-updated table");
-  if (opt.opt == HRB_OPT_FTRL) {
-    int rc = ftrl_tables_ok(plan, "hrb_lookup_bwd_update");
-    if (rc != HRB_OK) return rc;
-  }
-  const int G = plan->max_dim / 4;
-  if (G > 256) return fail(HRB_UNSUPPORTED, "hrb_lookup_bwd_update: dim %d too large", plan->max_dim);
-  if (batch == 0) return HRB_OK;
-  const int64_t n = batch * plan->pos_cols;
-  HRB_REQUIRE(n < 0x7FFFFFFFll, "hrb_lookup_bwd_update: batch*sum(seq_len) exceeds 2^31-1");
+  const char* who = "hrb_lookup_bwd_update";
+  int rc = bwd_check(plan, ids, dout, dout_ld, opt_host, workspace, batch, who);
+  if (rc != HRB_OK) return rc;
   cudaStream_t st = (cudaStream_t)stream;
-  float* pad_flags = nullptr;
-  if (opt.opt == HRB_OPT_FTRL && has_pooled(plan)) {
-    const size_t fb = pad_flag_bytes(plan);
-    if (workspace_bytes < fb) return fail(HRB_WORKSPACE, "hrb_lookup_bwd_update: workspace %zu < %zu bytes of padding flags", workspace_bytes, fb);
-    workspace_bytes = (workspace_bytes - fb) / 256 * 256;
-    pad_flags = (float*)((char*)workspace + workspace_bytes);
-    int rc = launch_pad_flags(plan, ids, ids_ld, batch, pad_flags, st);
-    if (rc != HRB_OK) return rc;
-  }
-  int rc = HRB_OK;
-  if (plan->bwd_algo != HRB_BWD_SORT && unit_path_supported(plan, batch))
-    rc = run_unit_update(plan, ids, ids_ld, batch, dout, dout_ld, opt, workspace, workspace_bytes, st);
-  else
-    rc = run_plan_sorted_update(plan, ids, ids_ld, batch, dout, dout_ld, opt, workspace, workspace_bytes, st);
-  if (rc != HRB_OK || pad_flags == nullptr) return rc;
-  return launch_ftrl_pad(plan, pad_flags, opt, st);
+  const bool pad = opt_host->opt == HRB_OPT_FTRL && has_pooled(plan);
+  rc = bwd_partition(plan, ids, ids_ld, batch, workspace, workspace_bytes, pad, who, st);
+  if (rc != HRB_OK) return rc;
+  return bwd_apply(plan, ids, ids_ld, batch, dout, dout_ld, opt_host, workspace, workspace_bytes, who, st);
 }
 
 static int run_plan_sorted_update(const hrb_plan* plan, const int32_t* ids, int64_t ids_ld, int64_t batch, const float* dout,
-                                  int64_t dout_ld, const hrb_opt_params& opt, void* workspace, size_t workspace_bytes, cudaStream_t st) {
+                                  int64_t dout_ld, const hrb_opt_params& opt, void* workspace, size_t workspace_bytes, const char* who,
+                                  cudaStream_t st) {
   const int G = plan->max_dim / 4;
   const int64_t n = batch * plan->pos_cols;
   BwdWorkspace w;
   int rc = carve_bwd_ws(n, batch * plan->n_fields + 1, plan->max_dim, plan->key_bits, workspace, w);
   if (rc != HRB_OK) return rc;
   if (w.total > workspace_bytes)
-    return fail(HRB_WORKSPACE, "hrb_lookup_bwd_update: workspace %zu < required %zu bytes", workspace_bytes, w.total);
+    return fail(HRB_WORKSPACE, "%s: workspace %zu < required %zu bytes", who, workspace_bytes, w.total);
   const uint32_t sentinel = (uint32_t)plan->total_rows;
   bwd_keys_kernel<<<grid_for(batch * plan->n_fields, 256), 256, 0, st>>>(plan->d_fields, plan->n_fields, plan->pos_cols,
                                                                         ids, ids_ld, batch, sentinel, w.keys_in,
diff --git a/handyrec_b200/csrc/plan.cuh b/handyrec_b200/csrc/plan.cuh
--- a/handyrec_b200/csrc/plan.cuh
+++ b/handyrec_b200/csrc/plan.cuh
@@ -217,6 +217,7 @@
   SliceGroupDev* d_groups = nullptr;
   TableSplitDev* d_splits = nullptr;
   TileDev* d_tiles = nullptr;
+  uint32_t* d_done = nullptr;
   int32_t n_units = 0, n_groups = 0, n_partials = 0, n_lists = 0, n_tiles = 0;
   int32_t g_values[8] = {0};
   int32_t g_unit_off[9] = {0};
@@ -262,12 +263,22 @@
   int32_t bwd_algo = 0;
   mutable std::mutex unit_mu;
   mutable hrb::UnitSet units;
+  struct BwdPartition {
+    int64_t batch = -1;
+    const void* workspace = nullptr;
+    size_t workspace_bytes = 0;
+    bool units = false;
+    bool pad = false;
+  };
+  mutable BwdPartition bwd_part;
 };
 
 
 namespace hrb {
 bool unit_path_supported(const hrb_plan* plan, int64_t batch);
 size_t unit_workspace_bytes(const hrb_plan* plan, int64_t batch);
-int run_unit_update(const hrb_plan* plan, const int32_t* ids, int64_t ids_ld, int64_t batch, const float* dout, int64_t dout_ld,
-                    const hrb_opt_params& opt, void* workspace, size_t workspace_bytes, cudaStream_t st);
-}
+int run_unit_partition(const hrb_plan* plan, const int32_t* ids, int64_t ids_ld, int64_t batch, void* workspace, size_t workspace_bytes,
+                       const char* who, cudaStream_t st);
+int run_unit_apply(const hrb_plan* plan, int64_t batch, const float* dout, int64_t dout_ld, const hrb_opt_params& opt, void* workspace,
+                   size_t workspace_bytes, const char* who, cudaStream_t st);
+}
diff --git a/handyrec_b200/engine.py b/handyrec_b200/engine.py
--- a/handyrec_b200/engine.py
+++ b/handyrec_b200/engine.py
@@ -320,12 +320,46 @@
     _bwd_trials: Optional[list] = None
     bwd_algo = "auto"
 
+    def _bwd_trial_step(self, B: int) -> bool:
+        return (self.autotune_embedding_bwd and self._marks is None and B == self.B and self.step_count >= 3 and len(self._bwd_trials or []) < 4
+                and self.bwd_algo == "auto")
+
+    early_bwd_partition = True
+    _early = False
+
+    def _issue_early_partition(self, ids: torch.Tensor, B: int) -> None:
+        self._early = False
+        if not self.early_bwd_partition or self._marks is not None or self._bwd_trial_step(B):
+            return
+        main = torch.cuda.current_stream()
+        if self._part_stream is None:
+            self._part_stream = torch.cuda.Stream()
+            self._step_start, self._lists_ready = torch.cuda.Event(), torch.cuda.Event()
+        self._step_start.record(main)
+        self._part_stream.wait_event(self._step_start)
+        with torch.cuda.stream(self._part_stream):
+            self._zero_table_grads()
+            self._mark_touched(self.plan, ids, range(len(self.tables)))
+            call("hrb_lookup_bwd_partition", self.plan._h, K._p(ids), ids.stride(0), B, K._p(self._ws_emb), self._ws_emb.numel(), K._stream())
+            self._mark("bwd_partition")
+            self._lists_ready.record(self._part_stream)
+        self._early = True
+
+    _part_stream = None
+
     def _embedding_backward(self, ids, B, st, op) -> None:
+        if self._early:
+            self._early = False
+            torch.cuda.current_stream().wait_event(self._lists_ready)
+            call("hrb_lookup_bwd_apply", self.plan._h, K._p(ids), ids.stride(0), B, K._p(self.dX0), self.K0p, None, ctypes.byref(op),
+                 K._p(self._ws_emb), self._ws_emb.numel(), st)
+            self._mark("embedding_bwd_update")
+            return
         self._zero_table_grads()
         self._mark_touched(self.plan, ids, range(len(self.tables)))
         trial = None
         n_trials = len(self._bwd_trials or [])
-        if self.autotune_embedding_bwd and self._marks is None and B == self.B and self.step_count >= 3 and n_trials < 4 and self.bwd_algo == "auto":
+        if self._bwd_trial_step(B):
             trial = _lib.BWD_UNITS if n_trials % 2 == 0 else _lib.BWD_SORT
             call("hrb_plan_set_bwd_algo", self.plan._h, trial)
             e0, e1 = torch.cuda.Event(enable_timing=True), torch.cuda.Event(enable_timing=True)
@@ -367,6 +401,7 @@
         B = ids.shape[0]
         st = K._stream()
         self.step_count += 1
+        self._issue_early_partition(ids, B)
         self.forward(ids, dense, training=True)
         self.loss_sum.zero_()
         dlogit = self.dZ[-1]
diff --git a/handyrec_b200/kernels.py b/handyrec_b200/kernels.py
--- a/handyrec_b200/kernels.py
+++ b/handyrec_b200/kernels.py
@@ -235,6 +235,24 @@
         call("hrb_lookup_bwd_workspace", self._h, self.ids_cols, batch, ctypes.byref(need))
         return need.value
 
+    def _bwd_workspace(self, B: int, workspace: Optional[torch.Tensor]) -> torch.Tensor:
+        if workspace is not None:
+            return workspace
+        need = self.workspace_bytes(B)
+        if self._ws is None or self._ws.numel() < need:
+            self._ws = torch.empty(need, device=self.device, dtype=torch.uint8)
+        return self._ws
+
+    @staticmethod
+    def opt_params(opt: str = "sgd", lr: float = 0.01, l2_scale: float = 0.0, beta1: float = 0.9, beta2: float = 0.999, eps: float = 1e-7,
+                   step: int = 1, l1: float = 0.0, l2: float = 0.0, lr_power: float = -0.5, l2_shrinkage: float = 0.0) -> OptParams:
+        op = OptParams()
+        op.opt = {"sgd": _lib.OPT_SGD, "adagrad": _lib.OPT_ADAGRAD, "ftrl": _lib.OPT_FTRL}.get(opt, _lib.OPT_ADAM_LAZY)
+        op.lr, op.beta1, op.beta2, op.eps, op.l2_scale = lr, beta1, beta2, eps, l2_scale
+        op.bias_corr1, op.bias_corr2 = 1.0 - beta1 ** step, 1.0 - beta2 ** step
+        op.l1, op.l2, op.lr_power, op.l2_shrinkage = l1, l2, lr_power, l2_shrinkage
+        return op
+
     def backward_update(self, ids: torch.Tensor, dout: torch.Tensor, opt: str = "sgd", lr: float = 0.01, l2_scale: float = 0.0,
                         beta1: float = 0.9, beta2: float = 0.999, eps: float = 1e-7, step: int = 1,
                         workspace: Optional[torch.Tensor] = None, autotune: bool = False, l1: float = 0.0, l2: float = 0.0,
@@ -242,16 +260,8 @@
         B = ids.shape[0]
         ids_ld = self._ids_ld(ids)
         dout_ld = _row_major_2d(_chk(dout, torch.float32, "dout", contiguous=False), "dout")
-        need = self.workspace_bytes(B)
-        if workspace is None:
-            if self._ws is None or self._ws.numel() < need:
-                self._ws = torch.empty(need, device=self.device, dtype=torch.uint8)
-            workspace = self._ws
-        op = OptParams()
-        op.opt = {"sgd": _lib.OPT_SGD, "adagrad": _lib.OPT_ADAGRAD, "ftrl": _lib.OPT_FTRL}.get(opt, _lib.OPT_ADAM_LAZY)
-        op.lr, op.beta1, op.beta2, op.eps, op.l2_scale = lr, beta1, beta2, eps, l2_scale
-        op.bias_corr1, op.bias_corr2 = 1.0 - beta1 ** step, 1.0 - beta2 ** step
-        op.l1, op.l2, op.lr_power, op.l2_shrinkage = l1, l2, lr_power, l2_shrinkage
+        workspace = self._bwd_workspace(B, workspace)
+        op = self.opt_params(opt, lr, l2_scale, beta1, beta2, eps, step, l1, l2, lr_power, l2_shrinkage)
         trial = self._next_bwd_trial(B) if autotune else None
         if trial is not None:
             call("hrb_plan_set_bwd_algo", self._h, _lib.BWD_UNITS if trial == "units" else _lib.BWD_SORT)
@@ -262,6 +272,18 @@
             e1.record()
             e1.synchronize()
             self._finish_bwd_trial(trial, e0.elapsed_time(e1))
+
+    def backward_partition(self, ids: torch.Tensor, workspace: Optional[torch.Tensor] = None) -> None:
+        B = ids.shape[0]
+        workspace = self._bwd_workspace(B, workspace)
+        call("hrb_lookup_bwd_partition", self._h, _p(ids), self._ids_ld(ids), B, _p(workspace), workspace.numel(), _stream())
+
+    def backward_apply(self, ids: torch.Tensor, dout: torch.Tensor, op: OptParams, workspace: Optional[torch.Tensor] = None) -> None:
+        B = ids.shape[0]
+        dout_ld = _row_major_2d(_chk(dout, torch.float32, "dout", contiguous=False), "dout")
+        workspace = self._bwd_workspace(B, workspace)
+        call("hrb_lookup_bwd_apply", self._h, _p(ids), self._ids_ld(ids), B, _p(dout), dout_ld, None, ctypes.byref(op), _p(workspace),
+             workspace.numel(), _stream())
 
     _bwd_trial_log = None
     bwd_algo = "auto"
diff --git a/handyrec_b200/sharded.py b/handyrec_b200/sharded.py
--- a/handyrec_b200/sharded.py
+++ b/handyrec_b200/sharded.py
@@ -259,6 +259,8 @@
 
 
 class ShardedDeepFMEngine(DeepFMEngine):
+
+    early_bwd_partition = False
 
     def __init__(self, tables, vocabs, fields, n_dense, comm, peer_ptrs=None, replicate_max_rows: int = 0, replicated=None,
                  p2p_grad_exchange: bool = True, **kw):
diff --git a/include/hrb200.h b/include/hrb200.h
--- a/include/hrb200.h
+++ b/include/hrb200.h
@@ -92,6 +92,11 @@
                           const float* dout, int64_t dout_ld, const float* inv_count,
                           const hrb_opt_params* opt_host, void* workspace, size_t workspace_bytes,
                           void* stream);
+int hrb_lookup_bwd_partition(const hrb_plan* plan, const int32_t* ids, int64_t ids_ld, int64_t batch, void* workspace,
+                             size_t workspace_bytes, void* stream);
+int hrb_lookup_bwd_apply(const hrb_plan* plan, const int32_t* ids, int64_t ids_ld, int64_t batch, const float* dout, int64_t dout_ld,
+                         const float* inv_count, const hrb_opt_params* opt_host, void* workspace, size_t workspace_bytes,
+                         void* stream);
 
 typedef enum hrb_bwd_algo { HRB_BWD_AUTO = 0, HRB_BWD_UNITS = 1, HRB_BWD_SORT = 2 } hrb_bwd_algo;
 int hrb_plan_set_bwd_algo(hrb_plan* plan, int32_t algo);
```

After: 55.14 million, median of 6. +2.6%, better.
